# solufast-cvprojects/multigriddet

Hardware: NVIDIA B200
Metric: encode+decode/NMS images/sec, COCO 608×608, 1–8 B200; % HBM peak (higher is better)
Workload: dtype f32

## Files before the change

include/mgd.h:

```cpp
#ifndef MGD_H_
#define MGD_H_

#ifdef __cplusplus
extern "C" {
#endif

#if defined(__GNUC__)
#define MGD_API __attribute__((visibility("default")))
#else
#define MGD_API
#endif

#define MGD_VERSION 100
#define MGD_MAX_LAYERS 5
#define MGD_MAX_ANCHORS_PER_LAYER 8

typedef enum {
    MGD_OK = 0,
    MGD_ERR_INVALID_ARGUMENT = 1,
    MGD_ERR_CLASS_RANGE = 2,
    MGD_ERR_CUDA = 3,
    MGD_ERR_NO_DEVICE = 4,
    MGD_ERR_UNSUPPORTED = 5
} mgd_status;

enum { MGD_MEM_HOST = 0, MGD_MEM_DEVICE = 1 };

enum {
    MGD_FLAG_SYNC = 1,
    MGD_FLAG_HOST_ZEROCOPY = 4,
    MGD_FLAG_TF_COMPAT = 2
};

enum { MGD_NMS_IOU = 0, MGD_NMS_DIOU = 1, MGD_NMS_SOFT = 2, MGD_NMS_WBF = 3 };
enum { MGD_WBF_CONF_AVG = 0, MGD_WBF_CONF_MAX = 1, MGD_WBF_CONF_BOX_AND_MODEL_AVG = 2 };

typedef struct {
    int num_layers;
    int num_classes;
    int input_h, input_w;
    int grid_h[MGD_MAX_LAYERS];
    int grid_w[MGD_MAX_LAYERS];
    int num_anchors[MGD_MAX_LAYERS];
    double anchors[MGD_MAX_LAYERS][MGD_MAX_ANCHORS_PER_LAYER][2];
    int anchors_f64;
} mgd_head_config;

typedef struct {
    int use_softmax;
    int rescore_confidence;
    double confidence;
    double nms_threshold;
    int nms_method;
    int per_class;
    int max_boxes;
    double soft_sigma;
    double soft_score_threshold;
} mgd_post_config;

MGD_API int mgd_version(void);
MGD_API const char *mgd_last_error(void);
MGD_API int mgd_device_count(void);

MGD_API int mgd_encode_targets(const mgd_head_config *cfg, const float *boxes,
                       int batch, int max_boxes, float *const *y_true,
                       int memory, int device, void *stream, int flags,
                       long long *stats);

MGD_API int mgd_decode_nms(const mgd_head_config *cfg, const mgd_post_config *post,
                   const float *const *preds, int batch, const int *image_hw,
                   double *boxes_xywh, int *boxes_xyxy, double *scores,
                   int *classes, int *index, int *counts,
                   int memory, int device, void *stream, int flags,
                   long long *stats);

MGD_API int mgd_encode_decode_nms(const mgd_head_config *cfg, const mgd_post_config *post,
                          const float *gt_boxes, int enc_batch, int max_gt_boxes,
                          float *const *y_true,
                          const float *const *preds, int dec_batch, const int *image_hw,
                          double *boxes_xywh, int *boxes_xyxy, double *scores,
                          int *classes, int *index, int *counts,
                          int device, void *stream, int flags);

MGD_API int mgd_decode_dense(const mgd_head_config *cfg, const mgd_post_config *post,
                     const float *const *preds, int batch, const int *image_hw,
                     double *out, int memory, int device, void *stream, int flags);

MGD_API int mgd_nms(const double *boxes, const double *scores, const int *classes, int n,
            double nms_threshold, int nms_method, int per_class, int max_keep,
            int *keep, int *n_keep, int memory, int device, void *stream, int flags);

MGD_API int mgd_wbf(const double *boxes, const double *scores, const int *classes,
            const double *box_weights, int n, double iou_thr, double skip_box_thr,
            int conf_type, double *out_boxes, double *out_scores, int *out_classes,
            int *n_out, int memory, int device, void *stream, int flags);

MGD_API int mgd_soft_nms(const double *boxes, const double *scores, int n, double sigma,
                 double score_threshold, int *keep, double *soft_scores, int *n_keep,
                 int memory, int device, void *stream, int flags);

enum { MGD_IOU_CORNER = 0, MGD_IOU_CENTRE = 1 };
MGD_API int mgd_match_detections(const double *det_boxes, const double *det_scores,
                         const int *det_classes, const int *det_counts, int batch, int max_dets,
                         const double *gt_boxes, const int *gt_classes, const int *gt_counts,
                         int max_gt, const double *iou_thresholds, int num_thresholds,
                         int iou_mode, unsigned char *tp, int *matched_gt,
                         int memory, int device, void *stream, int flags);

MGD_API int mgd_ignore_mask(const mgd_head_config *cfg, const float *const *y_pred,
                    const float *const *y_true, int batch, double ignore_thresh, double eps,
                    float *const *ignore_mask, float *const *assigned_anchor_iou,
                    float *const *max_iou_map, int memory, int device, void *stream, int flags);

MGD_API int mgd_encode_ignore_mask(const mgd_head_config *cfg, const float *boxes, int batch,
                           int max_boxes, const float *const *y_pred, float *const *y_true,
                           double ignore_thresh, double eps, float *const *ignore_mask,
                           float *const *assigned_anchor_iou, float *const *max_iou_map,
                           int device, void *stream, int flags);

enum { MGD_BOXES_I32 = 0, MGD_BOXES_F64 = 1 };
MGD_API int mgd_reshape_boxes(const void *boxes, int boxes_dtype, const int *counts,
                      const int *params, int batch, int max_boxes, void *out, float *out_f32,
                      int *out_counts, int memory, int device, void *stream, int flags);
MGD_API int mgd_mosaic_merge_boxes(const double *boxes, int num_sources, int max_boxes,
                           const int *params, int batch, int height, int width, double *out,
                           float *out_f32, int *out_counts,
                           int memory, int device, void *stream, int flags);

MGD_API int mgd_letterbox_boxes(const float *boxes, const int *counts, const int *params,
                        int batch, int max_in, int input_h, int input_w,
                        int max_boxes_per_image, int expansion, float *out,
                        int memory, int device, void *stream, int flags);

MGD_API int mgd_iou_matrix(const double *boxes1, int n, const double *boxes2, int m, double *out,
                   int memory, int device, void *stream, int flags);

MGD_API int mgd_poll_status(int device, void *stream);

#include <stddef.h>
MGD_API int mgd_host_alloc(size_t bytes, void **ptr);
MGD_API int mgd_host_free(void *ptr);

#define MGD_IPC_HANDLE_BYTES 64
typedef struct mgd_exchange mgd_exchange;
MGD_API int mgd_exchange_create(int device, int world_size, int rank, size_t bytes,
                        mgd_exchange **exchange, unsigned char *handle);
MGD_API int mgd_exchange_connect(mgd_exchange *exchange, const unsigned char *handles);
MGD_API int mgd_exchange_buffer(mgd_exchange *exchange, void **base, size_t *bytes);
MGD_API int mgd_exchange_timeouts(mgd_exchange *exchange, void *stream, int *timeouts);
MGD_API int mgd_exchange_destroy(mgd_exchange *exchange);

MGD_API int mgd_release_workspace(void);

#define MGD_PROFILE_KINDS 5
MGD_API int mgd_profile_begin(void);
MGD_API int mgd_profile_end(double *ms, long long *launches);

struct DLTensor;
MGD_API int mgd_encode_targets_dlpack(const mgd_head_config *cfg, const struct DLTensor *boxes,
                              struct DLTensor *const *y_true, void *stream, int flags,
                              long long *stats);
MGD_API int mgd_decode_nms_dlpack(const mgd_head_config *cfg, const mgd_post_config *post,
                          const struct DLTensor *const *preds,
                          const struct DLTensor *image_hw,
                          struct DLTensor *boxes_xywh, struct DLTensor *boxes_xyxy,
                          struct DLTensor *scores, struct DLTensor *classes,
                          struct DLTensor *index, struct DLTensor *counts,
                          void *stream, int flags, long long *stats);

#ifdef __cplusplus
}
#endif
#endif
```

multigriddet_b200/_lib.py:

```python
from __future__ import annotations

import ctypes
import os

import numpy as np

_HERE = os.path.dirname(os.path.abspath(__file__))
LIB_PATH = os.path.join(_HERE, "libmgd.so")

MGD_MAX_LAYERS = 5
MGD_MAX_ANCHORS_PER_LAYER = 8
MEM_HOST, MEM_DEVICE = 0, 1
FLAG_SYNC = 1
FLAG_TF_COMPAT = 2
FLAG_HOST_ZEROCOPY = 4
NMS_IOU, NMS_DIOU, NMS_SOFT, NMS_WBF = 0, 1, 2, 3
IOU_CORNER, IOU_CENTRE = 0, 1
BOXES_I32, BOXES_F64 = 0, 1

OK, ERR_INVALID_ARGUMENT, ERR_CLASS_RANGE, ERR_CUDA, ERR_NO_DEVICE, ERR_UNSUPPORTED = range(6)


class HeadConfig(ctypes.Structure):
    _fields_ = [
        ("num_layers", ctypes.c_int),
        ("num_classes", ctypes.c_int),
        ("input_h", ctypes.c_int),
        ("input_w", ctypes.c_int),
        ("grid_h", ctypes.c_int * MGD_MAX_LAYERS),
        ("grid_w", ctypes.c_int * MGD_MAX_LAYERS),
        ("num_anchors", ctypes.c_int * MGD_MAX_LAYERS),
        ("anchors", ((ctypes.c_double * 2) * MGD_MAX_ANCHORS_PER_LAYER) * MGD_MAX_LAYERS),
        ("anchors_f64", ctypes.c_int),
    ]


class PostConfig(ctypes.Structure):
    _fields_ = [
        ("use_softmax", ctypes.c_int),
        ("rescore_confidence", ctypes.c_int),
        ("confidence", ctypes.c_double),
        ("nms_threshold", ctypes.c_double),
        ("nms_method", ctypes.c_int),
        ("per_class", ctypes.c_int),
        ("max_boxes", ctypes.c_int),
        ("soft_sigma", ctypes.c_double),
        ("soft_score_threshold", ctypes.c_double),
    ]


class MgdError(RuntimeError):
    pass


_lib = None

_FP = ctypes.POINTER(ctypes.c_float)
_DP = ctypes.POINTER(ctypes.c_double)
_IP = ctypes.POINTER(ctypes.c_int)
_LLP = ctypes.POINTER(ctypes.c_longlong)

EXPORTS = ("mgd_version", "mgd_last_error", "mgd_device_count", "mgd_encode_targets",
           "mgd_decode_nms", "mgd_decode_dense", "mgd_nms", "mgd_soft_nms", "mgd_wbf", "mgd_poll_status",
           "mgd_encode_targets_dlpack", "mgd_decode_nms_dlpack", "mgd_profile_begin",
           "mgd_profile_end", "mgd_match_detections", "mgd_iou_matrix", "mgd_host_alloc",
           "mgd_host_free", "mgd_release_workspace", "mgd_reshape_boxes", "mgd_mosaic_merge_boxes",
           "mgd_ignore_mask", "mgd_encode_decode_nms", "mgd_letterbox_boxes",
           "mgd_encode_ignore_mask", "mgd_exchange_create", "mgd_exchange_connect",
           "mgd_exchange_buffer", "mgd_exchange_timeouts", "mgd_exchange_destroy")

IPC_HANDLE_BYTES = 64


def load():
    global _lib
    if _lib is not None:
        return _lib
    if not os.path.isfile(LIB_PATH):
        raise MgdError(
            f"{LIB_PATH} not found: build it with `python -m multigriddet_b200.build` "
            "(needs nvcc).  multigriddet_b200 has no CPU fallback.")
    lib = ctypes.CDLL(LIB_PATH)
    lib.mgd_version.restype = ctypes.c_int
    lib.mgd_last_error.restype = ctypes.c_char_p
    lib.mgd_device_count.restype = ctypes.c_int
    lib.mgd_encode_targets.restype = ctypes.c_int
    lib.mgd_encode_targets.argtypes = [
        ctypes.POINTER(HeadConfig), ctypes.c_void_p, ctypes.c_int, ctypes.c_int,
        ctypes.POINTER(ctypes.c_void_p), ctypes.c_int, ctypes.c_int, ctypes.c_void_p,
        ctypes.c_int, _LLP]
    lib.mgd_decode_nms.restype = ctypes.c_int
    lib.mgd_decode_nms.argtypes = [
        ctypes.POINTER(HeadConfig), ctypes.POINTER(PostConfig),
        ctypes.POINTER(ctypes.c_void_p), ctypes.c_int, ctypes.c_void_p,
        ctypes.c_void_p, ctypes.c_void_p, ctypes.c_void_p, ctypes.c_void_p, ctypes.c_void_p,
        ctypes.c_void_p, ctypes.c_int, ctypes.c_int, ctypes.c_void_p, ctypes.c_int, _LLP]
    lib.mgd_encode_decode_nms.restype = ctypes.c_int
    lib.mgd_encode_decode_nms.argtypes = [
        ctypes.POINTER(HeadConfig), ctypes.POINTER(PostConfig),
        ctypes.c_void_p, ctypes.c_int, ctypes.c_int, ctypes.POINTER(ctypes.c_void_p),
        ctypes.POINTER(ctypes.c_void_p), ctypes.c_int, ctypes.c_void_p,
        ctypes.c_void_p, ctypes.c_void_p, ctypes.c_void_p, ctypes.c_void_p, ctypes.c_void_p,
        ctypes.c_void_p, ctypes.c_int, ctypes.c_void_p, ctypes.c_int]
    lib.mgd_decode_dense.restype = ctypes.c_int
    lib.mgd_decode_dense.argtypes = [
        ctypes.POINTER(HeadConfig), ctypes.POINTER(PostConfig),
        ctypes.POINTER(ctypes.c_void_p), ctypes.c_int, ctypes.c_void_p, ctypes.c_void_p,
        ctypes.c_int, ctypes.c_int, ctypes.c_void_p, ctypes.c_int]
    lib.mgd_nms.restype = ctypes.c_int
    lib.mgd_nms.argtypes = [
        ctypes.c_void_p, ctypes.c_void_p, ctypes.c_void_p, ctypes.c_int, ctypes.c_double,
        ctypes.c_int, ctypes.c_int, ctypes.c_int, ctypes.c_void_p, ctypes.c_void_p,
        ctypes.c_int, ctypes.c_int, ctypes.c_void_p, ctypes.c_int]
    lib.mgd_wbf.restype = ctypes.c_int
    lib.mgd_wbf.argtypes = [
        ctypes.c_void_p, ctypes.c_void_p, ctypes.c_void_p, ctypes.c_void_p, ctypes.c_int,
        ctypes.c_double, ctypes.c_double, ctypes.c_int, ctypes.c_void_p, ctypes.c_void_p,
        ctypes.c_void_p, ctypes.c_void_p, ctypes.c_int, ctypes.c_int, ctypes.c_void_p, ctypes.c_int]
    lib.mgd_soft_nms.restype = ctypes.c_int
    lib.mgd_soft_nms.argtypes = [
        ctypes.c_void_p, ctypes.c_void_p, ctypes.c_int, ctypes.c_double, ctypes.c_double,
        ctypes.c_void_p, ctypes.c_void_p, ctypes.c_void_p, ctypes.c_int, ctypes.c_int,
        ctypes.c_void_p, ctypes.c_int]
    lib.mgd_poll_status.restype = ctypes.c_int
    lib.mgd_poll_status.argtypes = [ctypes.c_int, ctypes.c_void_p]
    lib.mgd_encode_targets_dlpack.restype = ctypes.c_int
    lib.mgd_encode_targets_dlpack.argtypes = [
        ctypes.POINTER(HeadConfig), ctypes.c_void_p, ctypes.POINTER(ctypes.c_void_p),
        ctypes.c_void_p, ctypes.c_int, _LLP]
    lib.mgd_decode_nms_dlpack.restype = ctypes.c_int
    lib.mgd_decode_nms_dlpack.argtypes = [
        ctypes.POINTER(HeadConfig), ctypes.POINTER(PostConfig),
        ctypes.POINTER(ctypes.c_void_p), ctypes.c_void_p, ctypes.c_void_p, ctypes.c_void_p,
        ctypes.c_void_p, ctypes.c_void_p, ctypes.c_void_p, ctypes.c_void_p, ctypes.c_void_p,
        ctypes.c_int, _LLP]
    lib.mgd_match_detections.restype = ctypes.c_int
    lib.mgd_match_detections.argtypes = [
        ctypes.c_void_p, ctypes.c_void_p, ctypes.c_void_p, ctypes.c_void_p, ctypes.c_int, ctypes.c_int,
        ctypes.c_void_p, ctypes.c_void_p, ctypes.c_void_p, ctypes.c_int, _DP, ctypes.c_int,
        ctypes.c_int, ctypes.c_void_p, ctypes.c_void_p, ctypes.c_int, ctypes.c_int, ctypes.c_void_p,
        ctypes.c_int]
    lib.mgd_iou_matrix.restype = ctypes.c_int
    lib.mgd_iou_matrix.argtypes = [
        ctypes.c_void_p, ctypes.c_int, ctypes.c_void_p, ctypes.c_int, ctypes.c_void_p, ctypes.c_int,
        ctypes.c_int, ctypes.c_void_p, ctypes.c_int]
    lib.mgd_reshape_boxes.restype = ctypes.c_int
    lib.mgd_reshape_boxes.argtypes = [
        ctypes.c_void_p, ctypes.c_int, ctypes.c_void_p, ctypes.c_void_p, ctypes.c_int, ctypes.c_int,
        ctypes.c_void_p, ctypes.c_void_p, ctypes.c_void_p, ctypes.c_int, ctypes.c_int, ctypes.c_void_p,
        ctypes.c_int]
    lib.mgd_mosaic_merge_boxes.restype = ctypes.c_int
    lib.mgd_mosaic_merge_boxes.argtypes = [
        ctypes.c_void_p, ctypes.c_int, ctypes.c_int, ctypes.c_void_p, ctypes.c_int, ctypes.c_int,
        ctypes.c_int, ctypes.c_void_p, ctypes.c_void_p, ctypes.c_void_p, ctypes.c_int, ctypes.c_int,
        ctypes.c_void_p, ctypes.c_int]
    lib.mgd_encode_ignore_mask.restype = ctypes.c_int
    lib.mgd_encode_ignore_mask.argtypes = [
        ctypes.POINTER(HeadConfig), ctypes.c_void_p, ctypes.c_int, ctypes.c_int,
        ctypes.POINTER(ctypes.c_void_p), ctypes.POINTER(ctypes.c_void_p), ctypes.c_double, ctypes.c_double,
        ctypes.POINTER(ctypes.c_void_p), ctypes.POINTER(ctypes.c_void_p), ctypes.POINTER(ctypes.c_void_p),
        ctypes.c_int, ctypes.c_void_p, ctypes.c_int]
    lib.mgd_letterbox_boxes.restype = ctypes.c_int
    lib.mgd_letterbox_boxes.argtypes = [
        ctypes.c_void_p, ctypes.c_void_p, ctypes.c_void_p, ctypes.c_int, ctypes.c_int, ctypes.c_int,
        ctypes.c_int, ctypes.c_int, ctypes.c_int, ctypes.c_void_p, ctypes.c_int, ctypes.c_int,
        ctypes.c_void_p, ctypes.c_int]
    lib.mgd_ignore_mask.restype = ctypes.c_int
    lib.mgd_ignore_mask.argtypes = [
        ctypes.POINTER(HeadConfig), ctypes.POINTER(ctypes.c_void_p), ctypes.POINTER(ctypes.c_void_p),
        ctypes.c_int, ctypes.c_double, ctypes.c_double, ctypes.POINTER(ctypes.c_void_p),
        ctypes.POINTER(ctypes.c_void_p), ctypes.POINTER(ctypes.c_void_p), ctypes.c_int, ctypes.c_int,
        ctypes.c_void_p, ctypes.c_int]
    lib.mgd_host_alloc.restype = ctypes.c_int
    lib.mgd_host_alloc.argtypes = [ctypes.c_size_t, ctypes.POINTER(ctypes.c_void_p)]
    lib.mgd_host_free.restype = ctypes.c_int
    lib.mgd_host_free.argtypes = [ctypes.c_void_p]
    lib.mgd_release_workspace.restype = ctypes.c_int
    lib.mgd_exchange_create.restype = ctypes.c_int
    lib.mgd_exchange_create.argtypes = [ctypes.c_int, ctypes.c_int, ctypes.c_int, ctypes.c_size_t,
                                        ctypes.POINTER(ctypes.c_void_p), ctypes.c_void_p]
    lib.mgd_exchange_connect.restype = ctypes.c_int
    lib.mgd_exchange_connect.argtypes = [ctypes.c_void_p, ctypes.c_void_p]
    lib.mgd_exchange_buffer.restype = ctypes.c_int
    lib.mgd_exchange_buffer.argtypes = [ctypes.c_void_p, ctypes.POINTER(ctypes.c_void_p),
                                        ctypes.POINTER(ctypes.c_size_t)]
    lib.mgd_exchange_timeouts.restype = ctypes.c_int
    lib.mgd_exchange_timeouts.argtypes = [ctypes.c_void_p, ctypes.c_void_p, _IP]
    lib.mgd_exchange_destroy.restype = ctypes.c_int
    lib.mgd_exchange_destroy.argtypes = [ctypes.c_void_p]
    lib.mgd_profile_begin.restype = ctypes.c_int
    lib.mgd_profile_end.restype = ctypes.c_int
    lib.mgd_profile_end.argtypes = [_DP, _LLP]
    _lib = lib
    return lib


def raise_for_status(rc: int) -> None:
    if rc == OK:
        return
    msg = load().mgd_last_error().decode("utf-8", "replace")
    if rc == ERR_CLASS_RANGE:
        raise AssertionError(msg)
    if rc == ERR_INVALID_ARGUMENT:
        raise ValueError(msg)
    if rc == ERR_UNSUPPORTED:
        raise NotImplementedError(msg)
    raise MgdError(msg)


_cfg_cache: dict = {}


def make_head_config(anchors, num_classes, input_shape, grid_shapes=None) -> HeadConfig:
    arrs = [np.asarray(a) for a in anchors]
    key = (tuple((a.dtype.str, a.shape, a.tobytes()) for a in arrs), int(num_classes),
           int(input_shape[0]), int(input_shape[1]),
           None if grid_shapes is None else tuple((int(g[0]), int(g[1])) for g in grid_shapes))
    hit = _cfg_cache.get(key)
    if hit is not None:
        return hit
    cfg = _make_head_config(arrs, num_classes, input_shape, grid_shapes)
    if len(_cfg_cache) < 256:
        _cfg_cache[key] = cfg
    return cfg


def _make_head_config(arrs, num_classes, input_shape, grid_shapes=None) -> HeadConfig:
    num_layers = len(arrs)
    if not 1 <= num_layers <= MGD_MAX_LAYERS:
        raise ValueError(f"between 1 and {MGD_MAX_LAYERS} layers supported, got {num_layers}")
    cfg = HeadConfig()
    cfg.num_layers = num_layers
    cfg.num_classes = int(num_classes)
    cfg.input_h, cfg.input_w = int(input_shape[0]), int(input_shape[1])
    if grid_shapes is None:
        strides = (32, 16, 8, 4, 2)
        grid_shapes = [(cfg.input_h // strides[l], cfg.input_w // strides[l])
                       for l in range(num_layers)]
    f64 = False
    for l, a in enumerate(arrs):
        if a.ndim != 2 or a.shape[1] != 2 or not 1 <= a.shape[0] <= MGD_MAX_ANCHORS_PER_LAYER:
            raise ValueError(f"anchors[{l}] must have shape (1..{MGD_MAX_ANCHORS_PER_LAYER}, 2)")
        f64 = f64 or a.dtype == np.float64
        cfg.grid_h[l], cfg.grid_w[l] = int(grid_shapes[l][0]), int(grid_shapes[l][1])
        cfg.num_anchors[l] = a.shape[0]
        for i in range(a.shape[0]):
            cfg.anchors[l][i][0] = float(a[i, 0])
            cfg.anchors[l][i][1] = float(a[i, 1])
    cfg.anchors_f64 = int(f64)
    return cfg


def ptr_array(ptrs):
    return (ctypes.c_void_p * len(ptrs))(*[ctypes.c_void_p(int(p)) for p in ptrs])


class PinnedPool:

    def __init__(self, cap_bytes=None):
        import threading
        if cap_bytes is None:
            cap_bytes = int(os.environ.get("MGD_PINNED_CAP_MB", "4096")) << 20
        self._lock = threading.Lock()
        self._free = {}
        self._idle = 0
        self._total = 0
        self.cap_bytes = cap_bytes

    def _give_back(self, ptr, nbytes):
        with self._lock:
            self._free.setdefault(nbytes, []).append(ptr)
            self._idle += nbytes

    def _trim(self, need):
        victims = []
        with self._lock:
            for size in sorted(self._free, reverse=True):
                lst = self._free[size]
                while lst and self._total + need > self.cap_bytes:
                    victims.append(lst.pop())
                    self._idle -= size
                    self._total -= size
        for ptr in victims:
            load().mgd_host_free(ctypes.c_void_p(ptr))

    def empty(self, shape, dtype):
        import weakref
        dtype = np.dtype(dtype)
        nbytes = int(np.prod(shape, dtype=np.int64)) * dtype.itemsize
        if nbytes < (1 << 16):
            return np.empty(shape, dtype)
        ptr = None
        with self._lock:
            lst = self._free.get(nbytes)
            if lst:
                ptr = lst.pop()
                self._idle -= nbytes
        if ptr is None:
            if self._total + nbytes > self.cap_bytes:
                self._trim(nbytes)
            if self._total + nbytes > self.cap_bytes:
                return np.empty(shape, dtype)
            out = ctypes.c_void_p()
            if load().mgd_host_alloc(nbytes, ctypes.byref(out)) != OK or not out.value:
                return np.empty(shape, dtype)
            ptr = out.value
            with self._lock:
                self._total += nbytes
        buf = (ctypes.c_char * nbytes).from_address(ptr)
        weakref.finalize(buf, self._give_back, ptr, nbytes)
        return np.frombuffer(buf, dtype=dtype).reshape(shape)


pinned = PinnedPool()
```

multigriddet_b200/csrc/api.cu:

```cuda
#include <math.h>
#include <stdarg.h>
#include <stdio.h>
#include <string.h>

#include <chrono>
#include <functional>
#include <mutex>
#include <string>
#include <thread>
#include <vector>

#include "common.cuh"
#include "dlpack_abi.h"

namespace {

thread_local std::string t_error;

int fail(int code, const char* fmt, ...)
{
    char buf[512];
    va_list ap;
    va_start(ap, fmt);
    vsnprintf(buf, sizeof(buf), fmt, ap);
// ... 655 lines not shown
    {
        if (!s[0] && !s[1] && chunk[0].blocks.empty() && chunk[1].blocks.empty() &&
            call.blocks.empty() && !bounce[0] && !bounce[1]) return;
        for (int i = 0; i < 2; ++i) if (s[i]) cudaStreamSynchronize(s[i]);
        chunk[0].release(); chunk[1].release(); call.release();
        for (int i = 0; i < 2; ++i) {
            if (bounce[i]) cudaFreeHost(bounce[i]);
            if (bounce_done[i]) cudaEventDestroy(bounce_done[i]);
            if (ev[i]) cudaEventDestroy(ev[i]);
            if (s[i]) cudaStreamDestroy(s[i]);
        }
        cudaGetLastError();
    }
};
thread_local HostStreams t_streams[64];

int host_streams(int device, cudaStream_t** out, cudaEvent_t** ev, HostStreams** self = nullptr)
{
    HostStreams& hs = t_streams[device];
    if (self) *self = &hs;
    for (int i = 0; i < 2; ++i) {
        if (!hs.s[i]) CUDA_TRY(cudaStreamCreateWithFlags(&hs.s[i], cudaStreamNonBlocking));
        if (!hs.ev[i]) CUDA_TRY(cudaEventCreateWithFlags(&hs.ev[i], cudaEventDisableTiming));
    }
    *out = hs.s;
    if (ev) *ev = hs.ev;
    return MGD_OK;
}

bool is_pageable(const void* p)
{
    cudaPointerAttributes at;
    if (cudaPointerGetAttributes(&at, p) != cudaSuccess) { cudaGetLastError(); return true; }
    return at.type == cudaMemoryTypeUnregistered;
}

int host_copy_threads()
{
    static int n = -1;
    if (n < 0) {
        const char* e = getenv("MGD_HOST_COPY_THREADS");
        const int hw = (int)std::thread::hardware_concurrency();
        n = e ? atoi(e) : (hw >= 32 ? 8 : (hw >= 8 ? hw / 4 : 2));
        if (hw > 0 && n > hw) n = hw;
        if (n < 1) n = 1;
    }
    return n;
}

void parallel_copy(void* dst, const void* src, size_t bytes)
{
    const int n = bytes < (8u << 20) ? 1 : host_copy_threads();
    if (n == 1) { memcpy(dst, src, bytes); return; }
    const size_t part = ((bytes / n) + 4095) & ~(size_t)4095;
    std::vector<std::thread> workers;
    for (int i = 1; i < n; ++i) {
        const size_t off = (size_t)i * part;
        if (off >= bytes) break;
        const size_t len = off + part < bytes ? part : bytes - off;
        workers.emplace_back([=] { memcpy(static_cast<char*>(dst) + off, static_cast<const char*>(src) + off, len); });
    }
    memcpy(dst, src, part < bytes ? part : bytes);
    for (std::thread& t : workers) t.join();
}

int bounce_slot(HostStreams* hs, int slot, size_t bytes, unsigned char** out)
{
    if (hs->bounce_busy[slot]) {
        CUDA_TRY(cudaEventSynchronize(hs->bounce_done[slot]));
        hs->bounce_busy[slot] = false;
    }
    if (hs->bounce_cap[slot] < bytes) {
        if (hs->bounce[slot]) CUDA_TRY(cudaFreeHost(hs->bounce[slot]));
        hs->bounce[slot] = nullptr; hs->bounce_cap[slot] = 0;
        CUDA_TRY(cudaHostAlloc(reinterpret_cast<void**>(&hs->bounce[slot]), bytes, cudaHostAllocPortable));
        hs->bounce_cap[slot] = bytes;
    }
    if (!hs->bounce_done[slot]) CUDA_TRY(cudaEventCreateWithFlags(&hs->bounce_done[slot], cudaEventDisableTiming));
    *out = hs->bounce[slot];
    return MGD_OK;
}

template <typename T> T* mapped_alias(T* p, size_t bytes)
{
    if (!p || bytes == 0) return nullptr;
    const unsigned char* ends[2] = {reinterpret_cast<const unsigned char*>(p),
                                    reinterpret_cast<const unsigned char*>(p) + bytes - 1};
    void* dev = nullptr;
    for (int i = 0; i < 2; ++i) {
        cudaPointerAttributes at;
        if (cudaPointerGetAttributes(&at, ends[i]) != cudaSuccess) { cudaGetLastError(); return nullptr; }
        if (at.type != cudaMemoryTypeHost || !at.devicePointer) return nullptr;
        if (i == 0) dev = at.devicePointer;
    }
    return reinterpret_cast<T*>(dev);
}

int zerocopy_mode()
{
    static int v = -1;
    if (v < 0) { const char* e = getenv("MGD_HOST_ZEROCOPY"); v = e ? atoi(e) : 0; }
    return v;
}

int host_chunk(const HeadGeom& g, int batch)
{
    static long long mb = -1;
    if (mb < 0) { const char* e = getenv("MGD_HOST_CHUNK_MB"); mb = e && atoll(e) > 0 ? atoll(e) : 128; }
    long long per_image = 0;
    for (int l = 0; l < g.L; ++l) per_image += (long long)g.gh[l] * g.gw[l] * g.D[l] * 4;
    long long n = (mb << 20) / (per_image > 0 ? per_image : 1);
    if (n < 1) n = 1;
    if (n > batch) n = batch;
    return (int)n;
}

}

extern "C" {

int mgd_version(void) { return MGD_VERSION; }

const char* mgd_last_error(void) { return t_error.c_str(); }

int mgd_device_count(void) { return device_count_quiet(); }

int mgd_host_alloc(size_t bytes, void** ptr)
{
    if (!ptr) return fail(MGD_ERR_INVALID_ARGUMENT, "ptr is NULL");
    *ptr = nullptr;
    if (device_count_quiet() == 0)
        return fail(MGD_ERR_NO_DEVICE, "no CUDA device: page-locked memory is not available");
    CUDA_TRY(cudaHostAlloc(ptr, bytes ? bytes : 1, cudaHostAllocPortable));
    return MGD_OK;
}

int mgd_host_free(void* ptr)
{
    if (ptr) CUDA_TRY(cudaFreeHost(ptr));
    return MGD_OK;
}

int mgd_exchange_create(int device, int world_size, int rank, size_t bytes, mgd_exchange** out,
                        unsigned char* handle)
{
    if (!out || !handle) return fail(MGD_ERR_INVALID_ARGUMENT, "NULL argument");
    *out = nullptr;
    if (world_size < 1 || world_size > MGD_EXCHANGE_MAX_RANKS)
        return fail(MGD_ERR_UNSUPPORTED, "a detection exchange spans 1..%d ranks (one node), got %d",
                    MGD_EXCHANGE_MAX_RANKS, world_size);
    if (rank < 0 || rank >= world_size) return fail(MGD_ERR_INVALID_ARGUMENT, "rank %d outside [0, %d)", rank, world_size);
    if (bytes == 0) return fail(MGD_ERR_INVALID_ARGUMENT, "bytes must be > 0");
    int num_sms;
    DeviceScope dev_scope;
    int rc = prepare_device(device, &num_sms, &dev_scope);
    if (rc) return rc;
    static_assert(sizeof(cudaIpcMemHandle_t) == MGD_IPC_HANDLE_BYTES, "IPC handle size");
    mgd_exchange* ex = new mgd_exchange();
    ex->device = device;
    ex->world = world_size;
    ex->rank = rank;
    ex->bytes = (bytes + 255) & ~(size_t)255;
    void* p = nullptr;
    cudaError_t e = cudaMalloc(&p, MGD_EXCHANGE_HEADER_BYTES + ex->bytes);
    if (e == cudaSuccess) e = cudaMemset(p, 0, MGD_EXCHANGE_HEADER_BYTES + ex->bytes);
    if (e == cudaSuccess) e = cudaIpcGetMemHandle(&ex->handle, p);
    if (e != cudaSuccess) {
        if (p) cudaFree(p);
        delete ex;
        cudaGetLastError();
        return fail(MGD_ERR_CUDA, "exchange allocation failed: %s", cudaGetErrorString(e));
    }
    ex->alloc[rank] = static_cast<char*>(p);
    memcpy(handle, &ex->handle, MGD_IPC_HANDLE_BYTES);
    if (world_size == 1) {
        ex->connected = true;
        std::lock_guard<std::mutex> lock(g_exchange_mutex);
        g_exchanges.push_back(ex);
    }
    *out = ex;
    return MGD_OK;
}

int mgd_exchange_connect(mgd_exchange* ex, const unsigned char* handles)
{
    if (!ex || !handles) return fail(MGD_ERR_INVALID_ARGUMENT, "NULL argument");
    if (ex->connected) return MGD_OK;
    int num_sms;
    DeviceScope dev_scope;
    int rc = prepare_device(ex->device, &num_sms, &dev_scope);
    if (rc) return rc;
    for (int r = 0; r < ex->world; ++r) {
        if (r == ex->rank) continue;
        cudaIpcMemHandle_t h;
        memcpy(&h, handles + (size_t)r * MGD_IPC_HANDLE_BYTES, MGD_IPC_HANDLE_BYTES);
        void* p = nullptr;
        const cudaError_t e = cudaIpcOpenMemHandle(&p, h, cudaIpcMemLazyEnablePeerAccess);
        if (e != cudaSuccess) {
            for (int q = 0; q < r; ++q)
                if (q != ex->rank && ex->alloc[q]) { cudaIpcCloseMemHandle(ex->alloc[q]); ex->alloc[q] = nullptr; }
            cudaGetLastError();
            return fail(MGD_ERR_CUDA, "cannot map the exchange buffer of rank %d: %s (peer access over "
                        "NVLink / PCIe between the two devices is required)", r, cudaGetErrorString(e));
        }
        ex->alloc[r] = static_cast<char*>(p);
    }
    ex->connected = true;
    std::lock_guard<std::mutex> lock(g_exchange_mutex);
    g_exchanges.push_back(ex);
    return MGD_OK;
}

int mgd_exchange_buffer(mgd_exchange* ex, void** base, size_t* bytes)
{
    if (!ex || !base) return fail(MGD_ERR_INVALID_ARGUMENT, "NULL argument");
    *base = ex->alloc[ex->rank] + MGD_EXCHANGE_HEADER_BYTES;
    if (bytes) *bytes = ex->bytes;
    return MGD_OK;
}

int mgd_exchange_timeouts(mgd_exchange* ex, void* stream, int* timeouts)
{
    if (!ex || !timeouts) return fail(MGD_ERR_INVALID_ARGUMENT, "NULL argument");
    int num_sms;
    DeviceScope dev_scope;
    int rc = prepare_device(ex->device, &num_sms, &dev_scope);
    if (rc) return rc;
    unsigned v = 0;
    CUDA_TRY(cudaStreamSynchronize((cudaStream_t)stream));
    CUDA_TRY(cudaMemcpy(&v, reinterpret_cast<unsigned*>(ex->alloc[ex->rank]) + MGD_EXCHANGE_TIMEOUT_WORD,
                        sizeof(v), cudaMemcpyDeviceToHost));
    *timeouts = (int)v;
    return MGD_OK;
}

int mgd_exchange_destroy(mgd_exchange* ex)
{
    if (!ex) return MGD_OK;
    {
        std::lock_guard<std::mutex> lock(g_exchange_mutex);
        for (size_t i = 0; i < g_exchanges.size(); ++i)
            if (g_exchanges[i] == ex) { g_exchanges.erase(g_exchanges.begin() + i); break; }
    }
    int num_sms;
    DeviceScope dev_scope;
    if (prepare_device(ex->device, &num_sms, &dev_scope) == MGD_OK) {
        cudaDeviceSynchronize();
        for (int r = 0; r < ex->world; ++r) {
            if (!ex->alloc[r]) continue;
            if (r == ex->rank) cudaFree(ex->alloc[r]);
            else cudaIpcCloseMemHandle(ex->alloc[r]);
        }
        cudaGetLastError();
    }
    delete ex;
    return MGD_OK;
}

int mgd_release_workspace(void)
{
    int cur = 0;
    const bool have = cudaGetDevice(&cur) == cudaSuccess;
    for (int d = 0; d < 64; ++d) {
        HostStreams& hs = t_streams[d];
        if (hs.chunk[0].blocks.empty() && hs.chunk[1].blocks.empty() && hs.call.blocks.empty() &&
            !hs.bounce[0] && !hs.bounce[1]) continue;
        if (cudaSetDevice(d) != cudaSuccess) { cudaGetLastError(); continue; }
        for (int i = 0; i < 2; ++i) if (hs.s[i]) cudaStreamSynchronize(hs.s[i]);
        hs.chunk[0].release(); hs.chunk[1].release(); hs.call.release();
        for (int i = 0; i < 2; ++i) {
            if (hs.bounce[i]) cudaFreeHost(hs.bounce[i]);
            hs.bounce[i] = nullptr; hs.bounce_cap[i] = 0; hs.bounce_busy[i] = false;
        }
    }
    if (have) cudaSetDevice(cur);
    cudaGetLastError();
    return MGD_OK;
}

int mgd_profile_begin(void)
{
    for (ProfSpan& s : t_prof_spans) { cudaEventDestroy(s.t0); cudaEventDestroy(s.t1); }
    t_prof_spans.clear();
    t_prof_on = true;
    return MGD_OK;
}

int mgd_profile_end(double* ms, long long* launches)
{
    t_prof_on = false;
    for (int k = 0; k < PROF_KINDS; ++k) { if (ms) ms[k] = 0.0; if (launches) launches[k] = 0; }
    int rc = MGD_OK;
    for (ProfSpan& s : t_prof_spans) {
        float t = 0.f;
        cudaError_t e = cudaEventSynchronize(s.t1);
        if (e == cudaSuccess) e = cudaEventElapsedTime(&t, s.t0, s.t1);
        if (e != cudaSuccess) rc = fail(MGD_ERR_CUDA, "profile: %s", cudaGetErrorString(e));
        else { if (ms) ms[s.kind] += t; if (launches) launches[s.kind] += s.launches; }
        cudaEventDestroy(s.t0);
        cudaEventDestroy(s.t1);
    }
    t_prof_spans.clear();
    return rc;
}

int mgd_poll_status(int device, void* stream)
{
    int num_sms;
    DeviceScope dev_scope;
    int rc = prepare_device(device, &num_sms, &dev_scope);
    if (rc) return rc;
    CUDA_TRY(cudaStreamSynchronize((cudaStream_t)stream));
    int st = 0;
    if (t_deferred.word[device]) {
        CUDA_TRY(cudaMemcpy(&st, t_deferred.word[device], sizeof(int), cudaMemcpyDeviceToHost));
        if (st) CUDA_TRY(cudaMemset(t_deferred.word[device], 0, sizeof(int)));
    }
    return status_to_error(st);
}

int mgd_encode_targets(const mgd_head_config* cfg, const float* boxes, int batch, int max_boxes,
                       float* const* y_true, int memory, int device, void* stream, int flags,
                       long long* stats)
{
    nvtx_range nv_api("mgd_encode_targets");
    HeadGeom g;
    int rc = build_geom(cfg, &g);
    if (rc) return rc;
    if ((rc = check_memory_arg(memory))) return rc;
    if (batch < 0 || max_boxes < 0)
        return fail(MGD_ERR_INVALID_ARGUMENT, "batch and max_boxes must be >= 0");
    if (!y_true) return fail(MGD_ERR_INVALID_ARGUMENT, "y_true is NULL");
    for (int l = 0; l < g.L; ++l)
        if (!y_true[l] && batch > 0) return fail(MGD_ERR_INVALID_ARGUMENT, "y_true[%d] is NULL", l);
    if (!boxes && (long long)batch * max_boxes > 0)
        return fail(MGD_ERR_INVALID_ARGUMENT, "boxes is NULL");
    if (max_boxes > 65000)
        return fail(MGD_ERR_UNSUPPORTED, "max_boxes per image must be <= 65000, got %d", max_boxes);
    if ((long long)chunk_images(g, batch > 0 ? batch : 1) * max_boxes >= (1ll << 27))
        return fail(MGD_ERR_UNSUPPORTED, "batch chunk x max_boxes too large");
    int num_sms;
    DeviceScope dev_scope;
    if ((rc = prepare_device(device, &num_sms, &dev_scope))) return rc;
    if (stats) memset(stats, 0, 4 * sizeof(long long));
    if (batch == 0) return MGD_OK;

    if (memory == MGD_MEM_DEVICE && !(flags & MGD_FLAG_SYNC)) {
        cudaStream_t st = (cudaStream_t)stream;
        int* d_flag;
        if ((rc = deferred_status_word(device, &d_flag))) return rc;
        return encode_device(g, boxes, batch, max_boxes, y_true, num_sms, st, d_flag, nullptr,
                             Alloc{nullptr, st}, (flags & MGD_FLAG_TF_COMPAT) != 0);
    }
    if (memory == MGD_MEM_DEVICE) {
        cudaStream_t st = (cudaStream_t)stream;
        int* d_status;
        unsigned long long* d_stats = nullptr;
        CUDA_TRY(pool_malloc(&d_status, sizeof(int) + 4 * sizeof(unsigned long long), st));
        CUDA_TRY(cudaMemsetAsync(d_status, 0, sizeof(int) + 4 * sizeof(unsigned long long), st));
        d_stats = reinterpret_cast<unsigned long long*>(d_status);
        int* d_flag = reinterpret_cast<int*>(d_stats + 4);
        rc = encode_device(g, boxes, batch, max_boxes, y_true, num_sms, st, d_flag, d_stats,
                           Alloc{nullptr, st}, (flags & MGD_FLAG_TF_COMPAT) != 0);
        if (rc) return rc;
        if (flags & MGD_FLAG_SYNC) {
            unsigned long long h[5] = {0, 0, 0, 0, 0};
            CUDA_TRY(cudaMemcpyAsync(h, d_status, sizeof(int) + 4 * sizeof(unsigned long long),
                                     cudaMemcpyDeviceToHost, st));
            CUDA_TRY(cudaFreeAsync(d_status, st));
            CUDA_TRY(cudaStreamSynchronize(st));
            if (stats) for (int i = 0; i < 4; ++i) stats[i] = (long long)h[i];
            return status_to_error((int)(h[4] & 0xffffffffu));
        }
        CUDA_TRY(cudaFreeAsync(d_status, st));
        return MGD_OK;
    }

    Tracer tr("encode/host");
    cudaStream_t* ss;
    cudaEvent_t* ev;
    HostStreams* hs;
    if ((rc = host_streams(device, &ss, &ev, &hs))) return rc;
    hs->call.reset();
    unsigned long long* d_meta;
    CUDA_TRY(hs->call.take(reinterpret_cast<void**>(&d_meta), 5 * sizeof(unsigned long long)));
    CUDA_TRY(cudaMemsetAsync(d_meta, 0, 5 * sizeof(unsigned long long), ss[0]));
    float* d_boxes;
    const size_t box_bytes = (size_t)batch * max_boxes * 5 * sizeof(float);
    CUDA_TRY(hs->call.take(reinterpret_cast<void**>(&d_boxes), box_bytes));
    if (box_bytes) CUDA_TRY(cudaMemcpyAsync(d_boxes, boxes, box_bytes, cudaMemcpyHostToDevice, ss[0]));
    CUDA_TRY(cudaEventRecord(ev[0], ss[0]));
    CUDA_TRY(cudaStreamWaitEvent(ss[1], ev[0], 0));
    int step = host_chunk(g, batch);
    float* z_y[MGD_MAX_LAYERS];
    bool zero_copy = (zerocopy_mode() & 2) != 0 || (flags & MGD_FLAG_HOST_ZEROCOPY) != 0;
    for (int l = 0; l < g.L && zero_copy; ++l) {
        z_y[l] = mapped_alias(y_true[l], (size_t)batch * g.gh[l] * g.gw[l] * g.D[l] * 4);
        zero_copy = z_y[l] != nullptr;
    }
    if (zero_copy) step = batch;
    bool pageable = !zero_copy && host_copy_threads() > 1 &&
                    (size_t)batch * g.cells * g.D[0] * 4 >= (32u << 20);
    for (int l = 0; l < g.L && pageable; ++l) pageable = is_pageable(y_true[l]);
    struct CopyOut { bool live = false; size_t off[MGD_MAX_LAYERS], bytes[MGD_MAX_LAYERS]; float* dst[MGD_MAX_LAYERS]; };
    CopyOut pending[2];
    auto drain = [&](int slot) -> int {
        CopyOut& c = pending[slot];
        if (!c.live) return MGD_OK;
        CUDA_TRY(cudaEventSynchronize(hs->bounce_done[slot]));
        hs->bounce_busy[slot] = false;
        for (int l = 0; l < g.L; ++l) parallel_copy(c.dst[l], hs->bounce[slot] + c.off[l], c.bytes[l]);
        c.live = false;
        return MGD_OK;
    };
    int k = 0;
    for (int b0 = 0; b0 < batch; b0 += step, ++k) {
        const int nb = batch - b0 < step ? batch - b0 : step;
        cudaStream_t st = ss[k & 1];
        Arena& ar = hs->chunk[k & 1];
        ar.reset();
        float* d_y[MGD_MAX_LAYERS];
        for (int l = 0; l < g.L; ++l) {
            if (zero_copy) d_y[l] = z_y[l];
            else CUDA_TRY(ar.take(reinterpret_cast<void**>(&d_y[l]), (size_t)nb * g.gh[l] * g.gw[l] * g.D[l] * 4));
        }
        rc = encode_device(g, d_boxes + (size_t)b0 * max_boxes * 5, nb, max_boxes, d_y, num_sms, st,
                           reinterpret_cast<int*>(d_meta + 4), d_meta, Alloc{&ar, st},
                           (flags & MGD_FLAG_TF_COMPAT) != 0);
        if (rc) return rc;
        unsigned char* bounce = nullptr;
        if (pageable) {
            if ((rc = drain(k & 1))) return rc;
            size_t need = 0;
            for (int l = 0; l < g.L; ++l) need += (((size_t)nb * g.gh[l] * g.gw[l] * g.D[l] * 4) + 255) & ~(size_t)255;
            if ((rc = bounce_slot(hs, k & 1, need, &bounce))) return rc;
        }
        size_t bounce_off = 0;
        for (int l = 0; l < g.L && !zero_copy; ++l) {
            const size_t per = (size_t)g.gh[l] * g.gw[l] * g.D[l];
            const size_t bytes = (size_t)nb * per * 4;
            float* dst = y_true[l] + (size_t)b0 * per;
            if (bounce) {
                CopyOut& c = pending[k & 1];
                c.off[l] = bounce_off; c.bytes[l] = bytes; c.dst[l] = dst;
                dst = reinterpret_cast<float*>(bounce + bounce_off);
                bounce_off += (bytes + 255) & ~(size_t)255;
            }
            CUDA_TRY(cudaMemcpyAsync(dst, d_y[l], bytes, cudaMemcpyDeviceToHost, st));
        }
        if (bounce) {
            CUDA_TRY(cudaEventRecord(hs->bounce_done[k & 1], st));
            hs->bounce_busy[k & 1] = true;
            pending[k & 1].live = true;
        }
    }
    if (pageable) {
        if ((rc = drain(k & 1))) return rc;
        if ((rc = drain((k + 1) & 1))) return rc;
    }
    tr.mark("chunks enqueued");
    CUDA_TRY(cudaEventRecord(ev[1], ss[1]));
    CUDA_TRY(cudaStreamWaitEvent(ss[0], ev[1], 0));
    CUDA_TRY(cudaStreamSynchronize(ss[0]));
    unsigned long long h[5];
    CUDA_TRY(cudaMemcpy(h, d_meta, sizeof(h), cudaMemcpyDeviceToHost));
    tr.mark("synchronised");
    hs->chunk[0].consolidate(); hs->chunk[1].consolidate(); hs->call.consolidate();
    if (stats) for (int i = 0; i < 4; ++i) stats[i] = (long long)h[i];
    return status_to_error((int)(h[4] & 0xffffffffu));
}

int mgd_decode_nms(const mgd_head_config* cfg, const mgd_post_config* post,
                   const float* const* preds, int batch, const int* image_hw,
                   double* boxes_xywh, int* boxes_xyxy, double* scores, int* classes, int* index,
                   int* counts, int memory, int device, void* stream, int flags, long long* stats)
{
    nvtx_range nv_api("mgd_decode_nms");
    HeadGeom g;
    int rc = build_geom(cfg, &g);
    if (rc) return rc;
    if ((rc = check_post(post))) return rc;
    if ((rc = check_memory_arg(memory))) return rc;
    if (batch < 0) return fail(MGD_ERR_INVALID_ARGUMENT, "batch must be >= 0");
    if (!preds) return fail(MGD_ERR_INVALID_ARGUMENT, "preds is NULL");
    for (int l = 0; l < g.L; ++l)
        if (!preds[l] && batch > 0) return fail(MGD_ERR_INVALID_ARGUMENT, "preds[%d] is NULL", l);
    if (!counts && batch > 0) return fail(MGD_ERR_INVALID_ARGUMENT, "counts is NULL");
    int num_sms;
    DeviceScope dev_scope;
    if ((rc = prepare_device(device, &num_sms, &dev_scope))) return rc;
    if (stats) memset(stats, 0, 4 * sizeof(long long));
    if (batch == 0) return MGD_OK;
    const int M = post->max_boxes;

    if (memory == MGD_MEM_DEVICE) {
        cudaStream_t st = (cudaStream_t)stream;
        unsigned long long* d_stats = nullptr;
        const bool want_stats = stats && (flags & MGD_FLAG_SYNC);
        if (want_stats) {
            CUDA_TRY(pool_malloc(&d_stats, 4 * sizeof(unsigned long long), st));
            CUDA_TRY(cudaMemsetAsync(d_stats, 0, 4 * sizeof(unsigned long long), st));
        }
        rc = decode_nms_device(g, *post, preds, batch, image_hw, boxes_xywh, boxes_xyxy, scores,
                               classes, index, counts, num_sms, st, d_stats, Alloc{nullptr, st});
        if (rc) return rc;
        if (flags & MGD_FLAG_SYNC) {
            unsigned long long h[4] = {0, 0, 0, 0};
            if (want_stats) {
                CUDA_TRY(cudaMemcpyAsync(h, d_stats, sizeof(h), cudaMemcpyDeviceToHost, st));
                CUDA_TRY(cudaFreeAsync(d_stats, st));
            }
            CUDA_TRY(cudaStreamSynchronize(st));
            if (stats) for (int i = 0; i < 4; ++i) stats[i] = (long long)h[i];
        }
        return MGD_OK;
    }

    Tracer tr("decode_nms/host");
    cudaStream_t* ss;
    cudaEvent_t* ev;
    HostStreams* hs;
    if ((rc = host_streams(device, &ss, &ev, &hs))) return rc;
    tr.mark("streams");
    const size_t n_det = (size_t)batch * M;
    const size_t off_xywh = 4 * sizeof(unsigned long long);
    const size_t off_scores = off_xywh + n_det * 4 * sizeof(double);
    const size_t off_xyxy = off_scores + n_det * sizeof(double);
    const size_t off_cls = off_xyxy + n_det * 4 * sizeof(int);
    const size_t off_idx = off_cls + n_det * sizeof(int);
    const size_t off_cnt = off_idx + n_det * sizeof(int);
    const size_t off_hw = off_cnt + (size_t)batch * sizeof(int);
    const size_t slab = off_hw + (size_t)batch * 2 * sizeof(int);
    unsigned char* d_out;
    hs->call.reset();
    CUDA_TRY(hs->call.take(reinterpret_cast<void**>(&d_out), slab));
    unsigned long long* d_stats = reinterpret_cast<unsigned long long*>(d_out);
    CUDA_TRY(cudaMemsetAsync(d_stats, 0, 4 * sizeof(unsigned long long), ss[0]));
    int* d_hw = nullptr;
    if (image_hw) {
        d_hw = reinterpret_cast<int*>(d_out + off_hw);
        CUDA_TRY(cudaMemcpyAsync(d_hw, image_hw, (size_t)batch * 2 * sizeof(int), cudaMemcpyHostToDevice, ss[0]));
    }
    CUDA_TRY(cudaEventRecord(ev[0], ss[0]));
    CUDA_TRY(cudaStreamWaitEvent(ss[1], ev[0], 0));
    tr.mark("slab");
    int step = host_chunk(g, batch);
    const float* z_pred[MGD_MAX_LAYERS];
    bool zero_copy = (zerocopy_mode() & 1) != 0 || (flags & MGD_FLAG_HOST_ZEROCOPY) != 0;
    for (int l = 0; l < g.L && zero_copy; ++l) {
        z_pred[l] = mapped_alias(preds[l], (size_t)batch * g.gh[l] * g.gw[l] * g.D[l] * 4);
        zero_copy = z_pred[l] != nullptr;
    }
    bool pageable = !zero_copy && host_copy_threads() > 1 &&
                    (size_t)batch * g.cells * g.D[0] * 4 >= (32u << 20);
    for (int l = 0; l < g.L && pageable; ++l) pageable = is_pageable(preds[l]);
    int k = 0;
    for (int b0 = 0; b0 < batch; b0 += step, ++k) {
        const int nb = batch - b0 < step ? batch - b0 : step;
        cudaStream_t st = ss[k & 1];
        Arena& ar = hs->chunk[k & 1];
        ar.reset();
        float* d_pred[MGD_MAX_LAYERS];
        unsigned char* bounce = nullptr;
        size_t bounce_off = 0;
        if (pageable) {
            size_t need = 0;
            for (int l = 0; l < g.L; ++l) need += (((size_t)nb * g.gh[l] * g.gw[l] * g.D[l] * 4) + 255) & ~(size_t)255;
            if ((rc = bounce_slot(hs, k & 1, need, &bounce))) return rc;
        }
        for (int l = 0; l < g.L; ++l) {
            const size_t per = (size_t)g.gh[l] * g.gw[l] * g.D[l];
            if (zero_copy) { d_pred[l] = const_cast<float*>(z_pred[l]) + (size_t)b0 * per; continue; }
            const size_t bytes = (size_t)nb * per * 4;
            CUDA_TRY(ar.take(reinterpret_cast<void**>(&d_pred[l]), bytes));
            const void* src = preds[l] + (size_t)b0 * per;
            if (bounce) {
                parallel_copy(bounce + bounce_off, src, bytes);
                src = bounce + bounce_off;
                bounce_off += (bytes + 255) & ~(size_t)255;
            }
            CUDA_TRY(cudaMemcpyAsync(d_pred[l], src, bytes, cudaMemcpyHostToDevice, st));
        }
        if (bounce) {
            CUDA_TRY(cudaEventRecord(hs->bounce_done[k & 1], st));
            hs->bounce_busy[k & 1] = true;
        }
        rc = decode_nms_device(g, *post, d_pred, nb, d_hw ? d_hw + 2 * (size_t)b0 : nullptr,
                               reinterpret_cast<double*>(d_out + off_xywh) + (size_t)b0 * M * 4,
                               reinterpret_cast<int*>(d_out + off_xyxy) + (size_t)b0 * M * 4,
                               reinterpret_cast<double*>(d_out + off_scores) + (size_t)b0 * M,
                               reinterpret_cast<int*>(d_out + off_cls) + (size_t)b0 * M,
                               reinterpret_cast<int*>(d_out + off_idx) + (size_t)b0 * M,
                               reinterpret_cast<int*>(d_out + off_cnt) + b0, num_sms, st, d_stats,
                               Alloc{&ar, st});
        if (rc) return rc;
    }
    tr.mark("chunks enqueued");
    CUDA_TRY(cudaEventRecord(ev[1], ss[1]));
    CUDA_TRY(cudaStreamWaitEvent(ss[0], ev[1], 0));
    cudaStream_t st = ss[0];
    CUDA_TRY(cudaStreamSynchronize(st));
    unsigned long long h[4];
    CUDA_TRY(cudaMemcpyAsync(h, d_stats, sizeof(h), cudaMemcpyDeviceToHost, st));
    if (boxes_xywh)
        CUDA_TRY(cudaMemcpyAsync(boxes_xywh, d_out + off_xywh, n_det * 4 * sizeof(double), cudaMemcpyDeviceToHost, st));
    if (scores)
// ... 927 lines not shown
```

multigriddet_b200/csrc/common.cuh:

```cuda
#pragma once
#include <cuda_runtime.h>
#include <stdint.h>
#include "../../include/mgd.h"

#define MGD_MAX_TOTAL_ANCHORS (MGD_MAX_LAYERS * MGD_MAX_ANCHORS_PER_LAYER)

struct HeadGeom {
    int L, C;
    int in_h, in_w;
    int gh[MGD_MAX_LAYERS], gw[MGD_MAX_LAYERS];
    int na[MGD_MAX_LAYERS];
    int D[MGD_MAX_LAYERS];
    int anchor_first[MGD_MAX_LAYERS];
    int K;
    int cell_off[MGD_MAX_LAYERS];
    int cells;
    int anchors_f64;
    float anc32[MGD_MAX_TOTAL_ANCHORS][2];
    double anc64[MGD_MAX_TOTAL_ANCHORS][2];
};

struct __align__(16) BoxRec {
    double fx, fy;
    float tw, th;
    int hot_anchor;
    int hot_class;
};

struct EncodeArgs {
    HeadGeom g;
    int B, N;
    const float* boxes;
    float* y[MGD_MAX_LAYERS];
    int* table;
    int* big_tables;
    BoxRec* recs;
    int tf_compat;
    int* status;
    unsigned long long* stats;
};

struct __align__(16) Cand {
    float score;
    int index;
    float t[4];
    int cls;
    int anchor;
};

struct __align__(16) BoxD { double x, y, w, h; };

struct DecodeArgs {
    HeadGeom g;
    int B;
    const float* pred[MGD_MAX_LAYERS];
    const int* image_hw;
    int use_softmax, rescore;
    double confidence;
    float obj_logit_min;
    float score_lo;
    long long rows_in_layer[MGD_MAX_LAYERS];
    unsigned long long cells_magic[MGD_MAX_LAYERS];
    Cand* cand;
    int* counts;
    int chunk_blocks;
    int debug;
};

#define MGD_MAX_MIRRORS 7
struct NmsArgs {
    HeadGeom g;
    int B;
    int cap;
    const Cand* cand;
    const double* in_boxes;
    const double* in_scores;
    const int* in_classes;
    BoxD* boxes;
    const int* counts;
    const int* image_hw;
    int in_h, in_w;
    double thr;
    int use_diou, per_class, max_boxes;
    int skip_small;
    int soft;
    double soft_sigma, soft_thr;
    double* soft_scratch;
    int wbf;
    int wbf_conf_type;
    const double* in_weights;
    int* wbf_ints;
    int* next_image;
    unsigned long long* sort_scratch;
    int sort_scratch_stride;
    unsigned char* kept_scratch;
    size_t kept_scratch_stride;
    double* out_xywh; int* out_xyxy; double* out_scores; int* out_classes; int* out_index;
    int* out_counts;
    unsigned long long* stats;
    int n_mirrors;
    long long mirror_delta[MGD_MAX_MIRRORS];
    int warp_ctas_per_sm;
};

#define MGD_EXCHANGE_MAX_RANKS 8
#define MGD_EXCHANGE_HEADER_BYTES 512
#define MGD_EXCHANGE_TIMEOUT_WORD 32
struct ExchangeView {
    int world, rank;
    unsigned* header[MGD_EXCHANGE_MAX_RANKS];
};
enum { MGD_EXCHANGE_SIGNAL = 1, MGD_EXCHANGE_WAIT = 2 };
cudaError_t launch_exchange_barrier(const ExchangeView& v, int which, unsigned epoch, int phase,
                                    cudaStream_t stream);

#define MGD_MAX_IOU_THRESHOLDS 16
struct MatchArgs {
    int B, M, N, T;
    const double* det_boxes;
    const double* det_scores;
    const int* det_classes;
    const int* det_counts;
    const double* gt_boxes;
    const int* gt_classes;
    const int* gt_counts;
    double thr[MGD_MAX_IOU_THRESHOLDS];
    int mode;
    unsigned char* tp;
    int* matched;
    int* next_image;
};

struct BoxOpArgs {
    int B, N;
    const void* in;
    const int* counts;
    const int* params;
    int n_src, height, width;
    void* out;
    float* out_f32;
    int* out_counts;
};

struct LossArgs {
    HeadGeom g;
    int B;
    const float* y_pred[MGD_MAX_LAYERS];
    const float* y_true[MGD_MAX_LAYERS];
    float ignore_thresh, eps;
    float* ignore[MGD_MAX_LAYERS];
    float* assigned[MGD_MAX_LAYERS];
    float* max_iou[MGD_MAX_LAYERS];
    void* gt_boxes;
    float* gt_area;
    int* gt_count;
    const int* table;
    const BoxRec* recs;
};

#include <nvtx3/nvToolsExt.h>
struct nvtx_range {
    explicit nvtx_range(const char* name) { nvtxRangePushA(name); }
    ~nvtx_range() { nvtxRangePop(); }
    nvtx_range(const nvtx_range&) = delete;
    nvtx_range& operator=(const nvtx_range&) = delete;
};

enum ProfKind { PROF_ENCODE_ASSIGN = 0, PROF_ENCODE_FILL = 1, PROF_DECODE_COMPACT = 2,
                PROF_NMS = 3, PROF_OTHER = 4, PROF_KINDS = 5 };
void prof_mark_begin(int kind, cudaStream_t stream);
void prof_mark_end(int kind, cudaStream_t stream);
void prof_group_begin(int kind, cudaStream_t stream);
void prof_group_end(int kind, cudaStream_t stream);

cudaError_t launch_encode(const EncodeArgs& a, int num_sms, cudaStream_t stream);
cudaError_t launch_encode_assign(const EncodeArgs& a, cudaStream_t stream,
                                 bool overlap_previous = false);
cudaError_t launch_encode_fill(const EncodeArgs& a, int num_sms, cudaStream_t stream,
                               bool overlap_previous = false);
cudaError_t launch_decode(const DecodeArgs& a, int num_sms, cudaStream_t stream);
cudaError_t launch_nms(const NmsArgs& a, int num_sms, cudaStream_t stream);
size_t encode_assign_smem_bytes(const HeadGeom& g, int N);
bool encode_needs_big_tables(const HeadGeom& g, int N);
int nms_smem_capacity();
size_t nms_kept_bytes(int max_boxes);
cudaError_t launch_decode_dense(const DecodeArgs& a, const int* image_hw, double* out,
                                cudaStream_t stream);
cudaError_t launch_match(const MatchArgs& a, int num_sms, cudaStream_t stream);
cudaError_t launch_iou_matrix(const double* b1, int n, const double* b2, int m, double* out,
                              cudaStream_t stream);
cudaError_t launch_reshape_boxes(const BoxOpArgs& a, int boxes_i32, cudaStream_t stream);
cudaError_t launch_mosaic_merge(const BoxOpArgs& a, cudaStream_t stream);
cudaError_t launch_letterbox_boxes(const float* in, const int* counts, const int* params, int B,
                                   int n_in, int n_keep, int capacity, int input_h, int input_w,
                                   float* out, cudaStream_t stream);
cudaError_t launch_ignore_mask(const LossArgs& a, cudaStream_t stream);
cudaError_t launch_keep_from_index(const int* index, const int* counts, int max_keep, int* keep,
                                   int* n_keep, cudaStream_t stream);
```

multigriddet_b200/csrc/decode.cu:

```cuda
#include <math.h>
#include <stdlib.h>
#include <string.h>
#include "common.cuh"
#include "decode_math.cuh"

namespace {

constexpr int kWarpsPerCta = 8;
constexpr int kThreads = kWarpsPerCta * 32;
constexpr int kDenseThreads = 256;

__device__ __forceinline__ uint32_t smem_u32(const void* p)
{
    return (uint32_t)__cvta_generic_to_shared(p);
}
__device__ __forceinline__ void mbar_init(uint64_t* bar, uint32_t count)
{
    asm volatile("mbarrier.init.shared::cta.b64 [%0], %1;" ::"r"(smem_u32(bar)), "r"(count));
}
__device__ __forceinline__ void fence_mbar_init()
{
    asm volatile("fence.mbarrier_init.release.cluster;" ::: "memory");
}
__device__ __forceinline__ void mbar_expect_tx(uint64_t* bar, uint32_t bytes)
// ... 30 lines not shown
    uint64_t* bar;
    int stride;
};

template <bool kFast, int kPoolRows>
__device__ __noinline__ void flush_pool(const DecodeArgs& a, const WarpPool& pool, int count,
                                        int layer, const uint64_t* s_tab)
{
    const HeadGeom& g = a.g;
    const int lane = threadIdx.x & 31;
    const int A = g.na[layer], C = g.C;
    const bool softmax = a.use_softmax != 0;
    const bool rescore = a.rescore != 0;

    bool pass = lane < count;
    if (pass && rescore) {
        const float* c = pool.rows + lane * pool.stride + 5 + A;
        float mc = -INFINITY, sum = 0.f;
        if (kFast) {
            const float4* c4 = reinterpret_cast<const float4*>(c);
            #pragma unroll 4
            for (int i = 0; i < C / 4; ++i) {
                const float4 v = c4[i];
                mc = fmaxf(fmaxf(mc, fmaxf(v.x, v.y)), fmaxf(v.z, v.w));
                if (softmax) sum += (fast_exp(v.x) + fast_exp(v.y)) + (fast_exp(v.z) + fast_exp(v.w));
            }
        } else {
            for (int i = 0; i < C; ++i) {
                mc = fmaxf(mc, c[i]);
                if (softmax) sum += fast_exp(c[i]);
            }
        }
        float ub;
        if (softmax) {
            ub = __fdividef(pool.bound[lane] * fast_exp(mc), sum);
            if (!(sum < 3.0e38f) || !(ub == ub)) ub = 3.0e38f;
        } else {
            ub = pool.bound[lane] * fast_sigmoid(mc);
        }
        pass = ub >= a.score_lo;
    }
    unsigned todo = __ballot_sync(0xffffffffu, pass);

    const int j = lane & 7;
    const int oct = lane >> 3;
    const unsigned omask = 0xffu << (oct * 8);
    const int cells_l = g.gh[layer] * g.gw[layer];
    while (todo) {
        const unsigned pos = nth_set_bit(todo, oct);
        if (pos < 32u) {
            float* x = pool.rows + pos * pool.stride;
            float pa, pc; int ka, kc;
            octet_probs(x + 5, A, j, omask, softmax, s_tab, pa, ka);
            octet_probs(x + 5 + A, C, j, omask, softmax, s_tab, pc, kc);
            float score = mgd_expitf_tab(x[4], s_tab);
            if (rescore) score = __fmul_rn(__fmul_rn(score, pa), pc);
            if (j == 0 && (double)score >= a.confidence) {
                const int grow = pool.cell[pos];
                const int b = grow / cells_l;
                const int cell = grow - b * cells_l;
                Cand cd;
                cd.score = score;
                cd.index = g.cell_off[layer] + cell;
                cd.t[0] = x[0]; cd.t[1] = x[1]; cd.t[2] = x[2]; cd.t[3] = x[3];
                cd.cls = kc;
                cd.anchor = g.anchor_first[layer] + ka;
                const int slot = atomicAdd(a.counts + b, 1);
                a.cand[(size_t)b * g.cells + slot] = cd;
            }
        }
        __syncwarp();
        #pragma unroll
        for (int q = 0; q < 4; ++q) todo &= todo - 1;
    }
    if (kFast) asm volatile("fence.proxy.async.shared::cta;" ::: "memory");
    __syncwarp();
}

template <bool kFast, int kPoolRows>
__global__ void __launch_bounds__(kThreads, kPoolRows >= 32 ? 2 : (kPoolRows >= 24 ? 3 : (kPoolRows >= 16 ? 4 : 2)))
decode_compact_kernel(const __grid_constant__ DecodeArgs a, int pool_stride)
{
    extern __shared__ __align__(128) unsigned char smem_raw[];
    __shared__ uint64_t s_bar[kWarpsPerCta];
    __shared__ uint64_t s_tab[MGD_EXP2F_N];
    __shared__ int s_cell[kWarpsPerCta][kPoolRows];
    __shared__ float s_bound[kWarpsPerCta][kPoolRows];

    const HeadGeom& g = a.g;
    const int tid = threadIdx.x;
    const int lane = tid & 31;
    const int warp = tid >> 5;
    WarpPool pool;
    pool.rows = reinterpret_cast<float*>(smem_raw) + (size_t)warp * kPoolRows * pool_stride;
    pool.cell = s_cell[warp];
    pool.bound = s_bound[warp];
    pool.bar = &s_bar[warp];
    pool.stride = pool_stride;

    if (tid < MGD_EXP2F_N) s_tab[tid] = mgd_exp2f_tab[tid];
    if (kFast && lane == 0) {
        mbar_init(pool.bar, 1);
        fence_mbar_init();
    }
    __syncthreads();

    const int gwarp = blockIdx.x * kWarpsPerCta + warp;
    const int n_warps = gridDim.x * kWarpsPerCta;
    const bool softmax = a.use_softmax != 0;
    const bool rescore = a.rescore != 0;
    uint32_t bar_phase = 0;

    for (int layer = 0; layer < g.L; ++layer) {
        const int D = g.D[layer];
        const int A = g.na[layer];
        const int n_rows = (int)a.rows_in_layer[layer];
        const int n_blocks = (n_rows + 31) >> 5;
        const float* base = a.pred[layer];
        int count = 0;

        auto load_head = [&](int blk, float4& q) {
            const int row = blk * 32 + lane;
            q = make_float4(NAN, 0.f, 0.f, 0.f);
            if (blk < n_blocks && row < n_rows) {
                if (kFast) q = __ldg(reinterpret_cast<const float4*>(base + (size_t)row * D + 4));
                else q.x = __ldg(base + (size_t)row * D + 4);
            }
        };
        float4 q_next;
        load_head(gwarp, q_next);
        for (int blk = gwarp; blk < n_blocks; blk += n_warps) {
            const float4 q = q_next;
            load_head(blk + n_warps, q_next);
            const int row = blk * 32 + lane;

            float bound = 0.f;
            bool pass = false;
            if (q.x >= a.obj_logit_min) {
                bound = fast_sigmoid(q.x);
                if (rescore) {
                    if (kFast) {
                        const float ma = fmaxf(q.y, fmaxf(q.z, q.w));
                        if (softmax)
                            bound = __fdividef(bound, (fast_exp(q.y - ma) + fast_exp(q.z - ma)) + fast_exp(q.w - ma));
                        else
                            bound *= fast_sigmoid(ma);
                    } else {
                        const float* an = base + (size_t)row * D + 5;
                        float ma = __ldg(an);
                        for (int i = 1; i < A; ++i) ma = fmaxf(ma, __ldg(an + i));
                        if (softmax) {
                            float sa = 0.f;
                            for (int i = 0; i < A; ++i) sa += fast_exp(__ldg(an + i) - ma);
                            bound = __fdividef(bound, sa);
                        } else {
                            bound *= fast_sigmoid(ma);
                        }
                    }
                }
                pass = bound >= a.score_lo;
            }
            unsigned todo = __ballot_sync(0xffffffffu, pass);
            if (!todo) continue;

            while (todo) {
                const int free_slots = kPoolRows - count;
                const int rank = __popc(todo & ((1u << lane) - 1u));
                const bool take = ((todo >> lane) & 1u) && rank < free_slots;
                const unsigned taken = __ballot_sync(0xffffffffu, take);
                const int n_new = __popc(taken);
                if (take) {
                    pool.cell[count + rank] = row;
                    pool.bound[count + rank] = bound;
                }
                if (kFast) {
                    if (lane == 0) mbar_expect_tx(pool.bar, (uint32_t)n_new * D * sizeof(float));
                    __syncwarp();
                    if (take)
                        bulk_g2s(pool.rows + (size_t)(count + rank) * pool.stride,
                                 base + (size_t)row * D, (uint32_t)D * sizeof(float), pool.bar);
                } else {
                    unsigned rest = taken;
                    int slot = count;
                    while (rest) {
                        const int src_lane = __ffs((int)rest) - 1;
                        rest &= rest - 1;
                        const float* src = base + ((size_t)blk * 32 + src_lane) * D;
                        float* dst = pool.rows + (size_t)slot * pool.stride;
                        for (int i = lane; i < D; i += 32) dst[i] = __ldg(src + i);
                        ++slot;
                    }
                    __syncwarp();
                }
                count += n_new;
                todo &= ~taken;
                if (count == kPoolRows) {
                    if (kFast) {
                        if (lane == 0) mbar_arrive(pool.bar);
                        mbar_wait(pool.bar, bar_phase);
                        bar_phase ^= 1u;
                    }
                    flush_pool<kFast, kPoolRows>(a, pool, count, layer, s_tab);
                    count = 0;
                }
            }
        }
        if (count) {
            if (kFast) {
                if (lane == 0) mbar_arrive(pool.bar);
                mbar_wait(pool.bar, bar_phase);
                bar_phase ^= 1u;
            }
            flush_pool<kFast, kPoolRows>(a, pool, count, layer, s_tab);
        }
        __syncwarp();
    }
}

namespace ws {

template <int kProducers_, int kConsumers_, int kSlots_, int kRows_ = 32, int kPrefetch_ = 16>
struct Shape {
    static constexpr int kPrefetch = kPrefetch_;
    static constexpr int kProducers = kProducers_;
    static constexpr int kConsumers = kConsumers_;
    static constexpr int kThreads = (kProducers_ + kConsumers_) * 32;
    static constexpr int kSlots = kSlots_;
    static constexpr int kRows = kRows_;
    static constexpr int kCtasPerSm = kSlots_ * kRows_ > 9 * 32 ? 1 : 2;
};
constexpr int kSlotRows = 32;

struct SlotMeta {
    int row[kSlotRows];
    float bound[kSlotRows];
    int count;
    int layer;
    int pad[2];
};

__device__ __forceinline__ float expf_core2(float x, const uint32_t* tab)
{
    const double inv_ln2_n = 0x1.71547652b82fep+0 * MGD_EXP2F_N;
    const double shift = 0x1.8p+52;
    const double c0 = 0x1.c6af84b912394p-5 / MGD_EXP2F_N / MGD_EXP2F_N / MGD_EXP2F_N;
    const double c1 = 0x1.ebfce50fac4f3p-3 / MGD_EXP2F_N / MGD_EXP2F_N;
    const double c2 = 0x1.62e42ff0c52d6p-1 / MGD_EXP2F_N;
    const double z = __dmul_rn(inv_ln2_n, (double)x);
    double kd = __dadd_rn(z, shift);
    const int ki = __double2loint(kd);
    kd = __dsub_rn(kd, shift);
    const double r = __fma_rn(inv_ln2_n, (double)x, -kd);
    const int idx = ki & (MGD_EXP2F_N - 1);
    const int hi = (int)tab[idx + MGD_EXP2F_N] + (ki << 15);
    const double sc = __hiloint2double(hi, (int)tab[idx]);
    const double q = __fma_rn(c0, r, c1);
    const double r2 = __dmul_rn(r, r);
    double y = __fma_rn(c2, r, 1.0);
    y = __fma_rn(q, r2, y);
    y = __dmul_rn(y, sc);
    return __double2float_rn(y);
}

__device__ __forceinline__ float expf_full2(float x, const uint32_t* tab)
{
    float special = 0.f;
    bool is_special = false;
    if (!(x < 88.0f && x > -88.0f)) {
        if (x != x) { special = x + x; is_special = true; }
        else if (x > 88.72283172607421875f) { special = __builtin_huge_valf(); is_special = true; }
        else if (x < -103.972076416015625f) { special = 0.0f; is_special = true; }
    }
    const float v = expf_core2(is_special ? 0.f : x, tab);
    return is_special ? special : v;
}

__device__ __forceinline__ void near_track(float d, float thr, int i, int& first, int& cnt)
{
    asm("{\n .reg .pred p;\n setp.ge.f32 p, %2, %3;\n @p min.s32 %0, %0, %4;\n @p add.s32 %1, %1, 1;\n}"
        : "+r"(first), "+r"(cnt) : "f"(d), "f"(thr), "r"(i));
}

__device__ __forceinline__ int ld_acquire_smem(const int* p)
{
    int v;
    asm volatile("ld.acquire.cta.shared.s32 %0, [%1];" : "=r"(v) : "r"(smem_u32(p)) : "memory");
    return v;
}
__device__ __forceinline__ void st_release_smem(int* p, int v)
{
    asm volatile("st.release.cta.shared.s32 [%0], %1;" ::"r"(smem_u32(p)), "r"(v) : "memory");
}

struct GroupShared {
    float4* stage;
    float* rows;
    SlotMeta* meta;
    uint64_t* full;
    int* published;
    int* released;
    int* fill_seq;
    int* next_seq;
    int* producers_done;
    int stride;
};

template <class Sh>
__device__ __forceinline__ void producer(const DecodeArgs& a, const GroupShared& gs, int p, int P)
{
    constexpr int kSlots = Sh::kSlots;
    constexpr int kRows = Sh::kRows;
    constexpr int kPrefetch = Sh::kPrefetch;
    constexpr int kConsumers = Sh::kConsumers;
    constexpr int kProducers = Sh::kProducers;
    const HeadGeom& g = a.g;
    const int lane = threadIdx.x & 31;
    const bool softmax = a.use_softmax != 0;
    const bool rescore = a.rescore != 0;
    int seq = 0, slot = 0, count = 0;
    bool have_slot = false;

    auto acquire = [&]() {
        if (lane == 0) {
            seq = atomicAdd(gs.fill_seq, 1);
            const int use = seq / kSlots;
            while (ld_acquire_smem(&gs.released[seq % kSlots]) != use) __nanosleep(40);
        }
        seq = __shfl_sync(0xffffffffu, seq, 0);
        slot = seq % kSlots;
        have_slot = true;
    };
    auto publish = [&](int cnt, int layer) {
        if (lane == 0) { gs.meta[slot].count = cnt; gs.meta[slot].layer = layer; }
        __syncwarp();
        if (lane == 0) {
            mbar_arrive(&gs.full[slot]);
            st_release_smem(&gs.published[slot], seq);
        }
        have_slot = false;
        count = 0;
    };

    for (int layer = 0; layer < g.L; ++layer) {
        const int D = g.D[layer];
        const int n_rows = (int)a.rows_in_layer[layer];
        const int n_blocks = (n_rows + 31) >> 5;
        const float* base = a.pred[layer];
        auto issue_head = [&](int blk, int st) {
            const int row = blk * 32 + lane;
            if (blk < n_blocks && row < n_rows)
                asm volatile("cp.async.cg.shared.global [%0], [%1], 16;"
                             ::"r"(smem_u32(gs.stage + st * 32 + lane)), "l"(base + (size_t)row * D + 4) : "memory");
            asm volatile("cp.async.commit_group;" ::: "memory");
        };
        const int kChunk = a.chunk_blocks;
        #pragma unroll
        for (int k = 0; k < kPrefetch; ++k) issue_head((p + (k / kChunk) * P) * kChunk + k % kChunk, k);
        auto stage_rows = [&](int blk, unsigned todo, float bound) {
            const int row = blk * 32 + lane;
            while (todo) {
                if (!have_slot) acquire();
                const int free_slots = kRows - count;
                const int rank = __popc(todo & ((1u << lane) - 1u));
                const bool take = ((todo >> lane) & 1u) && rank < free_slots;
                const unsigned taken = __ballot_sync(0xffffffffu, take);
                const int n_new = __popc(taken);
                if (take) {
                    gs.meta[slot].row[count + rank] = row;
                    gs.meta[slot].bound[count + rank] = bound;
                }
                if (lane == 0) mbar_expect_tx(&gs.full[slot], (uint32_t)n_new * D * sizeof(float));
                __syncwarp();
                if (take)
                    bulk_g2s(gs.rows + ((size_t)slot * kRows + count + rank) * gs.stride,
                             base + (size_t)row * D, (uint32_t)D * sizeof(float), &gs.full[slot]);
                count += n_new;
                todo &= ~taken;
                if (count == kRows) publish(count, layer);
            }
        };
        int st = 0;
        for (int chunk = p; chunk * kChunk < n_blocks; chunk += P) {
            for (int u = 0; u < kChunk; ++u) {
                const int blk = chunk * kChunk + u;
                asm volatile("cp.async.wait_group %0;" ::"n"(kPrefetch - 1) : "memory");
                const int row = blk * 32 + lane;
                float4 h = gs.stage[st * 32 + lane];
                if (row >= n_rows) h.x = NAN;
                issue_head(blk + kPrefetch * P, st);
                st = st + 1 == kPrefetch ? 0 : st + 1;

                float bound = 0.f;
                bool pass = false;
                if (h.x >= a.obj_logit_min) {
                    bound = fast_sigmoid(h.x);
                    if (rescore) {
                        const float ma = fmaxf(h.y, fmaxf(h.z, h.w));
                        if (softmax)
                            bound = __fdividef(bound, (fast_exp(h.y - ma) + fast_exp(h.z - ma)) + fast_exp(h.w - ma));
                        else
                            bound *= fast_sigmoid(ma);
                    }
                    pass = bound >= a.score_lo;
                }
                unsigned todo = __ballot_sync(0xffffffffu, pass);
                if (a.debug & 1) todo = 0;
                stage_rows(blk, todo, bound);
            }
        }
        if (count) publish(count, layer);
    }
    int done = 0;
    if (lane == 0) done = atomicAdd(gs.producers_done, 1) + 1;
    done = __shfl_sync(0xffffffffu, done, 0);
    if (done == kProducers)
        for (int c = 0; c < kConsumers; ++c) {
            acquire();
            publish(-1, 0);
        }
}

template <class Sh, int kC>
__device__ __forceinline__ void consumer(const DecodeArgs& a, const GroupShared& gs,
                                         const uint32_t* tab)
{
    constexpr int kSlots = Sh::kSlots;
    constexpr int kRows = Sh::kRows;
    constexpr int kSplit = 32 / kRows;
    const HeadGeom& g = a.g;
    const int lane = threadIdx.x & 31;
    const int j = lane & 7;
    const int oct = lane >> 3;
    const bool softmax = a.use_softmax != 0;
    const bool rescore = a.rescore != 0;
    const int C = kC ? kC : g.C;
    const int body = C >= 8 ? (C & ~7) : 0;
    const int tail = C - body;
    constexpr float kNear = 0.99999f;
    constexpr float kNearD = -1.1e-5f;

    for (;;) {
        int seq = 0;
        if (lane == 0) {
            seq = atomicAdd(gs.next_seq, 1);
            while (ld_acquire_smem(&gs.published[seq % kSlots]) != seq) __nanosleep(40);
        }
        seq = __shfl_sync(0xffffffffu, seq, 0);
        const int slot = seq % kSlots;
        mbar_wait(&gs.full[slot], ((unsigned)(seq / kSlots)) & 1u);
        const SlotMeta& meta = gs.meta[slot];
        const int count = meta.count;
        if (count < 0) break;
        const int layer = meta.layer;
        const float* rows = gs.rows + (size_t)slot * kRows * gs.stride;

        const int lrow = lane & (kRows - 1), part = lane / kRows;
        bool pass = lrow < count && !(a.debug & 4);
        float mc = -INFINITY, sum = 0.f;
        if (pass) {
            const float4* c4 = reinterpret_cast<const float4*>(rows + (size_t)lrow * gs.stride + 8);
            const int n4 = C / 4, per = (n4 + kSplit - 1) / kSplit;
            const int i0 = part * per, i1 = min(n4, i0 + per);
            if (softmax && rescore) {
                #pragma unroll 4
                for (int i = i0; i < i1; ++i) {
                    const float4 v = c4[i];
                    mc = fmaxf(fmaxf(mc, fmaxf(v.x, v.y)), fmaxf(v.z, v.w));
                    sum += (fast_exp(v.x) + fast_exp(v.y)) + (fast_exp(v.z) + fast_exp(v.w));
                }
            } else {
                #pragma unroll 4
                for (int i = i0; i < i1; ++i) {
                    const float4 v = c4[i];
                    mc = fmaxf(fmaxf(mc, fmaxf(v.x, v.y)), fmaxf(v.z, v.w));
                }
            }
        }
        if (kSplit == 2) {
            mc = fmaxf(mc, __shfl_xor_sync(0xffffffffu, mc, 16));
            sum += __shfl_xor_sync(0xffffffffu, sum, 16);
        }
        if (pass && rescore) {
            if (softmax) {
                float ub = __fdividef(meta.bound[lrow] * fast_exp(mc), sum);
                if (!(sum < 3.0e38f) || !(ub == ub)) ub = 3.0e38f;
                pass = ub >= a.score_lo;
            } else {
                pass = meta.bound[lrow] * fast_sigmoid(mc) >= a.score_lo;
            }
        }
        unsigned todo = __ballot_sync(0xffffffffu, pass) & (kRows == 32 ? 0xffffffffu : (1u << (kRows & 31)) - 1u);
        if (a.debug & 2) todo = 0;

        unsigned cand_rows = 0;
        while (todo) {
            const unsigned pos = nth_set_bit(todo, oct);
            const bool live = pos < 32u;
            const unsigned posr = live ? pos : (unsigned)__ffs((int)todo) - 1u;
            const float* x = rows + (size_t)posr * gs.stride;
            const float mx = __shfl_sync(0xffffffffu, mc, (int)posr);
            const float4 head = *reinterpret_cast<const float4*>(x + 4);
            const int l0 = oct * 8;
            float pa, pc, obj;
            int ka, kc;
            if (softmax) {
                const float ma = fmaxf(head.y, fmaxf(head.z, head.w));
                const float logit = x[5 + (j < 2 ? j : 2)];
                const float da = __fsub_rn(logit, ma);
                const float arg = j < 3 ? (da < -104.0f ? -104.0f : da) : (j == 3 ? -head.x : 0.f);
                const float ea = expf_full2(arg, tab);

                const float* cx = x + 8;
                float r = 0.f, e_tail = 0.f;
                int near_cnt = 0, near_first = INT_MAX;
                if (body) {
                    #pragma unroll 10
                    for (int i = j; i < body; i += 8) {
                        const float d = __fsub_rn(cx[i], mx);
                        const float e = expf_core2(d < -104.0f ? -104.0f : d, tab);
                        r = __fadd_rn(r, e);
                        near_track(d, kNearD, i, near_first, near_cnt);
                    }
                    r = __fadd_rn(r, __shfl_xor_sync(0xffffffffu, r, 1));
                    r = __fadd_rn(r, __shfl_xor_sync(0xffffffffu, r, 2));
                    r = __fadd_rn(r, __shfl_xor_sync(0xffffffffu, r, 4));
                }
                if (tail) {
                    if (j < tail) {
                        const float d = __fsub_rn(cx[body + j], mx);
                        e_tail = expf_core2(d < -104.0f ? -104.0f : d, tab);
                        near_track(d, kNearD, body + j, near_first, near_cnt);
                    }
                    for (int k = 0; k < tail; ++k)
                        r = __fadd_rn(r, __shfl_sync(0xffffffffu, e_tail, l0 + k));
                }
                pc = __frcp_rn(r);
                const float e0 = __shfl_sync(0xffffffffu, ea, l0);
                const float e1 = __shfl_sync(0xffffffffu, ea, l0 + 1);
                const float e2 = __shfl_sync(0xffffffffu, ea, l0 + 2);
                const float eo = __shfl_sync(0xffffffffu, ea, l0 + 3);
                const float sa = __fadd_rn(__fadd_rn(__fadd_rn(0.f, e0), e1), e2);
                pa = __frcp_rn(sa);
                obj = __frcp_rn(__fadd_rn(1.0f, eo));
                const unsigned has = (__ballot_sync(0xffffffffu, near_cnt > 0) >> l0) & 0xffu;
                const unsigned many = (__ballot_sync(0xffffffffu, near_cnt > 1) >> l0) & 0xffu;
                const bool simple = !many && __popc(has) == 1;
                kc = __shfl_sync(0xffffffffu, near_first, l0 + (has ? __ffs((int)has) - 1 : 0));
                const int n0 = e0 >= kNear, n1 = e1 >= kNear, n2 = e2 >= kNear;
                ka = n0 ? 0 : (n1 ? 1 : 2);
                if (__any_sync(0xffffffffu, !simple || n0 + n1 + n2 != 1)) {
                    int first = INT_MAX;
                    for (int i = j; i < C; i += 8) {
                        const float d = __fsub_rn(cx[i], mx);
                        const float e = expf_core2(d < -104.0f ? -104.0f : d, tab);
                        if (e >= kNear && __fdiv_rn(e, r) == pc) { first = i; break; }
                    }
                    first = min(first, __shfl_xor_sync(0xffffffffu, first, 1));
                    first = min(first, __shfl_xor_sync(0xffffffffu, first, 2));
                    first = min(first, __shfl_xor_sync(0xffffffffu, first, 4));
                    if (!simple) kc = first;
                    if (n0 + n1 + n2 != 1) {
                        ka = INT_MAX;
                        if (n2 && __fdiv_rn(e2, sa) == pa) ka = 2;
                        if (n1 && __fdiv_rn(e1, sa) == pa) ka = 1;
                        if (n0 && __fdiv_rn(e0, sa) == pa) ka = 0;
                    }
                }
            } else {
                float best = -INFINITY;
                int first = INT_MAX;
                for (int i = j; i < C; i += 8) {
                    const float qv = __fdiv_rn(1.0f, __fadd_rn(1.0f, expf_full2(-x[8 + i], tab)));
                    if (qv > best) { best = qv; first = i; }
                }
                #pragma unroll
                for (int d = 1; d <= 4; d <<= 1) {
                    const float ob = __shfl_xor_sync(0xffffffffu, best, d);
                    const int oi = __shfl_xor_sync(0xffffffffu, first, d);
                    if (ob > best || (ob == best && oi < first)) { best = ob; first = oi; }
                }
                pc = best; kc = first;
                const float logit = j == 0 ? head.x : (j == 1 ? head.y : (j == 2 ? head.z : head.w));
                const float qv = __fdiv_rn(1.0f, __fadd_rn(1.0f, expf_full2(-logit, tab)));
                obj = __shfl_sync(0xffffffffu, qv, l0);
                const float q0 = __shfl_sync(0xffffffffu, qv, l0 + 1);
                const float q1 = __shfl_sync(0xffffffffu, qv, l0 + 2);
                const float q2 = __shfl_sync(0xffffffffu, qv, l0 + 3);
                pa = -INFINITY; ka = INT_MAX;
                if (q0 > pa) { pa = q0; ka = 0; }
                if (q1 > pa) { pa = q1; ka = 1; }
                if (q2 > pa) { pa = q2; ka = 2; }
            }
            float score = obj;
            if (rescore) score = __fmul_rn(__fmul_rn(score, pa), pc);
            const bool is_cand = live && j == 0 && (double)score >= a.confidence;
            __syncwarp();
            if (is_cand) {
                float4 res;
                res.x = score;
                res.y = __int_as_float(kc);
                res.z = __int_as_float(g.anchor_first[layer] + ka);
                res.w = 0.f;
                *reinterpret_cast<float4*>(const_cast<float*>(x) + 4) = res;
            }
            cand_rows |= __reduce_or_sync(0xffffffffu, is_cand ? (1u << pos) : 0u);
            #pragma unroll
            for (int q = 0; q < 4; ++q) todo &= todo - 1;
        }
        __syncwarp();
        const bool mine = lane < kRows && ((cand_rows >> lane) & 1u);
        float4 t = make_float4(0.f, 0.f, 0.f, 0.f), res = t;
        unsigned grow = 0;
        if (mine) {
            const float* x = rows + (size_t)lane * gs.stride;
            t = *reinterpret_cast<const float4*>(x);
            res = *reinterpret_cast<const float4*>(x + 4);
            grow = (unsigned)meta.row[lane];
        }
        if (cand_rows) asm volatile("fence.proxy.async.shared::cta;" ::: "memory");
        __syncwarp();
        if (lane == 0) st_release_smem(&gs.released[slot], seq / kSlots + 1);
        if (cand_rows) {
            const unsigned long long magic = a.cells_magic[layer];
            const unsigned b = magic ? (unsigned)__umul64hi((unsigned long long)grow, magic) : grow;
            const unsigned same = __match_any_sync(0xffffffffu, mine ? b : (0x80000000u | (unsigned)lane));
            const int leader = __ffs((int)same) - 1;
            int base = 0;
            if (mine && lane == leader) base = atomicAdd(a.counts + b, __popc(same));
            base = __shfl_sync(0xffffffffu, base, leader);
            if (mine) {
                Cand cd;
                cd.score = res.x;
                cd.index = g.cell_off[layer] + (int)(grow - b * (unsigned)(g.gh[layer] * g.gw[layer]));
                cd.t[0] = t.x; cd.t[1] = t.y; cd.t[2] = t.z; cd.t[3] = t.w;
                cd.cls = __float_as_int(res.y);
                cd.anchor = __float_as_int(res.z);
                a.cand[(size_t)b * g.cells + base + __popc(same & ((1u << lane) - 1u))] = cd;
            }
        }
    }
}

template <class Sh, int kC>
__global__ void __launch_bounds__(Sh::kThreads, Sh::kCtasPerSm)
decode_ws_kernel(const __grid_constant__ DecodeArgs a, int stride)
{
    constexpr int kSlots = Sh::kSlots, kProducers = Sh::kProducers;
    extern __shared__ __align__(128) unsigned char smem_raw[];
    __shared__ uint64_t s_full[kSlots];
    __shared__ int s_published[kSlots], s_released[kSlots];
    __shared__ SlotMeta s_meta[kSlots];
    __shared__ uint32_t s_tab[2 * MGD_EXP2F_N];
    __shared__ int s_counters[3];


    const int tid = threadIdx.x;
    const int warp = tid >> 5;
    if (tid < MGD_EXP2F_N) {
        s_tab[tid] = (uint32_t)mgd_exp2f_tab[tid];
        s_tab[tid + MGD_EXP2F_N] = (uint32_t)(mgd_exp2f_tab[tid] >> 32);
    }
    if (tid == 0) {
        for (int sl = 0; sl < kSlots; ++sl) {
            mbar_init(&s_full[sl], 1);
            s_published[sl] = -1;
            s_released[sl] = 0;
        }
        s_counters[0] = s_counters[1] = s_counters[2] = 0;
        fence_mbar_init();
    }
    __syncthreads();

    GroupShared gs;
    gs.rows = reinterpret_cast<float*>(smem_raw);
    constexpr int kFirstProducer = Sh::kConsumers;
    const int pw = warp - kFirstProducer;
    gs.stage = reinterpret_cast<float4*>(gs.rows + (size_t)kSlots * Sh::kRows * stride) +
               (size_t)(pw >= 0 ? pw : 0) * Sh::kPrefetch * 32;
    gs.meta = s_meta;
    gs.full = s_full;
    gs.published = s_published;
    gs.released = s_released;
    gs.fill_seq = &s_counters[0];
    gs.next_seq = &s_counters[1];
    gs.producers_done = &s_counters[2];
    gs.stride = stride;
    if (pw >= 0)
        producer<Sh>(a, gs, blockIdx.x * kProducers + pw, gridDim.x * kProducers);
    else
        consumer<Sh, kC>(a, gs, s_tab);
}

}

__global__ void __launch_bounds__(kDenseThreads, 3)
decode_dense_kernel(const __grid_constant__ DecodeArgs a, const int* image_hw, double* out,
                    int row_floats)
{
    extern __shared__ __align__(128) unsigned char smem_raw[];
    __shared__ uint64_t s_tab[MGD_EXP2F_N];
    const HeadGeom& g = a.g;
    const int tid = threadIdx.x, j = tid & 7;
    const unsigned omask = 0xffu << (((tid & 31) >> 3) * 8);
    float* x = reinterpret_cast<float*>(smem_raw) + (size_t)(tid >> 3) * row_floats;
    if (tid < MGD_EXP2F_N) s_tab[tid] = mgd_exp2f_tab[tid];
    __syncthreads();
    const long long total_rows = (long long)a.B * g.cells;
    const long long octs = (long long)gridDim.x * (kDenseThreads / 8);
    const long long iters = (total_rows + octs - 1) / octs;
    for (long long it = 0; it < iters; ++it) {
        long long q = it * octs + (long long)blockIdx.x * (kDenseThreads / 8) + (tid >> 3);
        const bool live = q < total_rows;
        if (!live) q = total_rows - 1;
        const int b = (int)(q / g.cells);
        const int flat = (int)(q - (long long)b * g.cells);
        int layer = 0;
        while (layer + 1 < g.L && flat >= g.cell_off[layer + 1]) ++layer;
        const int cell = flat - g.cell_off[layer];
        const int D = g.D[layer], A = g.na[layer];
        const float* src = a.pred[layer] + ((size_t)b * g.gh[layer] * g.gw[layer] + cell) * D;
        for (int i = j; i < D; i += 8) x[i] = __ldg(src + i);
        __syncwarp(omask);
        float pa, pc; int ka, kc;
        octet_probs(x + 5, A, j, omask, a.use_softmax != 0, s_tab, pa, ka);
        octet_probs(x + 5 + A, g.C, j, omask, a.use_softmax != 0, s_tab, pc, kc);
        __syncwarp(omask);
        float score = mgd_expitf_tab(x[4], s_tab);
        if (a.rescore) score = __fmul_rn(__fmul_rn(score, pa), pc);
        const int rr = cell / g.gw[layer], cc = cell - rr * g.gw[layer];
        double box[4];
        Letterbox lb;
        if (image_hw) lb = letterbox_consts(g.in_h, g.in_w, image_hw[2 * b], image_hw[2 * b + 1]);
        decode_axis_of(g, x, layer, g.anchor_first[layer] + ka, rr, cc, image_hw ? &lb : nullptr, 0,
                       s_tab, box[0], box[2]);
        decode_axis_of(g, x, layer, g.anchor_first[layer] + ka, rr, cc, image_hw ? &lb : nullptr, 1,
                       s_tab, box[1], box[3]);
        if (live) {
            double* o = out + (size_t)q * (5 + g.C);
            if (j < 4) o[j] = box[j];
            if (j == 4) o[4] = (double)score;
            float s = 1.0f;
            if (a.use_softmax) s = np_sum_octet(x + 5 + A, g.C, j, omask);
            for (int i = j; i < g.C; i += 8) {
                const float e = x[5 + A + i];
                o[5 + i] = (double)(a.use_softmax ? __fdiv_rn(e, s) : e);
            }
        } else if (a.use_softmax) {
            (void)np_sum_octet(x + 5 + A, g.C, j, omask);
        }
        __syncwarp(omask);
    }
}

}

cudaError_t launch_decode(const DecodeArgs& a_in, int num_sms, cudaStream_t stream)
{
    DecodeArgs a = a_in;
    const HeadGeom& g = a.g;
    int dmax = 0;
    bool fast = true;
    for (int l = 0; l < g.L; ++l) {
        dmax = g.D[l] > dmax ? g.D[l] : dmax;
        fast = fast && g.na[l] == 3 && (g.D[l] % 4 == 0) &&
               ((reinterpret_cast<uintptr_t>(a.pred[l]) & 15) == 0);
        a.rows_in_layer[l] = (long long)a.B * g.gh[l] * g.gw[l];
        if (a.rows_in_layer[l] >= 0x7fffffffll - 64) return cudaErrorInvalidValue;
        const unsigned long long cells_l = (unsigned long long)g.gh[l] * g.gw[l];
        a.cells_magic[l] = cells_l > 1 ? ~0ull / cells_l + 1ull : 0ull;
    }
    int stride = fast ? (dmax / 4 | 1) * 4 : (dmax | 1);
    if (fast && stride < dmax) stride += 8;

    static int env_impl = -1;
    static int env_shape = 0;
    if (env_impl < 0) {
        const char* e = getenv("MGD_DECODE_IMPL");
        env_impl = e && !strcmp(e, "legacy") ? 1 : 0;
        const char* sh = getenv("MGD_DECODE_SHAPE");
        env_shape = sh ? atoi(sh) : 0;
    }
    static int env_debug = -1;
    if (env_debug < 0) { const char* e = getenv("MGD_DECODE_DEBUG"); env_debug = e ? atoi(e) : 0; }
    a.debug = env_debug;
    if (fast && g.C <= 128 && !env_impl) {
        long long blocks = 0;
        for (int l = 0; l < g.L; ++l) blocks += (a.rows_in_layer[l] + 31) / 32;
        const int ws_stride = dmax;
        auto run = [&](auto shape) -> cudaError_t {
            using Sh = decltype(shape);
            const size_t smem = (size_t)Sh::kSlots * Sh::kRows * ws_stride * sizeof(float) +
                                (size_t)Sh::kProducers * Sh::kPrefetch * 32 * sizeof(float4);
            const size_t fixed = 1024 + 1024 + (size_t)Sh::kSlots * 304;
            int ctas_per_sm = (int)((227 * 1024) / (smem + fixed));
            if (ctas_per_sm > Sh::kCtasPerSm) ctas_per_sm = Sh::kCtasPerSm;
            if (ctas_per_sm < 1) return cudaErrorInvalidConfiguration;
            long long grid = (long long)num_sms * ctas_per_sm;
            const long long needed = (blocks + Sh::kProducers * 4 - 1) / (Sh::kProducers * 4);
            if (grid > needed) grid = needed;
            if (grid < 1) grid = 1;
            const long long per_producer = blocks / (grid * Sh::kProducers);
            a.chunk_blocks = per_producer >= 768 ? 8 : (per_producer >= 64 ? 2 : 1);
            static int env_cb = -1;
            if (env_cb < 0) { const char* e = getenv("MGD_DECODE_CHUNK_BLOCKS"); env_cb = e ? atoi(e) : 0; }
            if (env_cb == 1 || env_cb == 2 || env_cb == 4 || env_cb == 8) a.chunk_blocks = env_cb;

            auto kernel = g.C == 80 ? ws::decode_ws_kernel<Sh, 80> : ws::decode_ws_kernel<Sh, 0>;
            cudaError_t e = cudaFuncSetAttribute(kernel, cudaFuncAttributeMaxDynamicSharedMemorySize, (int)smem);
            if (e != cudaSuccess) return e;
            prof_mark_begin(PROF_DECODE_COMPACT, stream);
            kernel<<<(unsigned)grid, Sh::kThreads, smem, stream>>>(a, ws_stride);
            prof_mark_end(PROF_DECODE_COMPACT, stream);
            return cudaGetLastError();
        };
        cudaError_t err;
        if (env_shape == 1) err = run(ws::Shape<3, 6, 17, 16, 8>());
        else if (env_shape == 3) err = run(ws::Shape<3, 8, 17, 16, 8>());
        else if (env_shape == 4) err = run(ws::Shape<3, 6, 7, 32>());
        else if (env_shape == 5) err = run(ws::Shape<2, 4, 8, 32>());
        else err = run(ws::Shape<3, 7, 17, 16, 8>());
        if (err != cudaErrorInvalidConfiguration) return err;
        cudaGetLastError();
    }
    static int env_pool = -1;
    if (env_pool < 0) { const char* e = getenv("MGD_DECODE_POOL_ROWS"); env_pool = e ? atoi(e) : 0; }
    int pool_rows = env_pool == 32 || env_pool == 24 || env_pool == 16 ? env_pool : 32;
    while (pool_rows > 16 && (size_t)kWarpsPerCta * pool_rows * stride * sizeof(float) > 200 * 1024) pool_rows -= 8;
    while (pool_rows > 4 && (size_t)kWarpsPerCta * pool_rows * stride * sizeof(float) > 200 * 1024) pool_rows /= 2;
    const size_t smem = (size_t)kWarpsPerCta * pool_rows * stride * sizeof(float);
    if (smem > 220 * 1024) return cudaErrorInvalidConfiguration;
    int ctas_per_sm = (int)((224 * 1024) / (smem + 2048));
    const int reg_limit = pool_rows >= 32 ? 2 : (pool_rows >= 24 ? 3 : (pool_rows >= 16 ? 4 : 2));
    if (ctas_per_sm > reg_limit) ctas_per_sm = reg_limit;
    if (ctas_per_sm < 1) ctas_per_sm = 1;
    long long blocks = 0;
    for (int l = 0; l < g.L; ++l) blocks += (a.rows_in_layer[l] + 31) / 32;
    long long grid = (long long)num_sms * ctas_per_sm;
    const long long needed = (blocks + kWarpsPerCta - 1) / kWarpsPerCta;
    if (grid > needed) grid = needed;
    if (grid < 1) grid = 1;
    cudaError_t err;
    prof_mark_begin(PROF_DECODE_COMPACT, stream);
    auto run = [&](auto kernel) -> cudaError_t {
        cudaError_t e = cudaFuncSetAttribute(kernel, cudaFuncAttributeMaxDynamicSharedMemorySize, (int)smem);
        if (e != cudaSuccess) return e;
        kernel<<<(unsigned)grid, kThreads, smem, stream>>>(a, stride);
        return cudaSuccess;
    };
    if (fast) {
        if (pool_rows == 32) err = run(decode_compact_kernel<true, 32>);
        else if (pool_rows == 24) err = run(decode_compact_kernel<true, 24>);
        else if (pool_rows == 16) err = run(decode_compact_kernel<true, 16>);
        else if (pool_rows == 8) err = run(decode_compact_kernel<true, 8>);
        else err = run(decode_compact_kernel<true, 4>);
    } else {
        if (pool_rows == 32) err = run(decode_compact_kernel<false, 32>);
        else if (pool_rows == 24) err = run(decode_compact_kernel<false, 24>);
        else if (pool_rows == 16) err = run(decode_compact_kernel<false, 16>);
        else if (pool_rows == 8) err = run(decode_compact_kernel<false, 8>);
        else err = run(decode_compact_kernel<false, 4>);
    }
    if (err != cudaSuccess) return err;
    prof_mark_end(PROF_DECODE_COMPACT, stream);
    return cudaGetLastError();
}

cudaError_t launch_decode_dense(const DecodeArgs& a, const int* image_hw, double* out,
                                cudaStream_t stream)
{
    const HeadGeom& g = a.g;
    int dmax = 0;
    for (int l = 0; l < g.L; ++l) dmax = g.D[l] > dmax ? g.D[l] : dmax;
    const int row_floats = (dmax + 3) & ~3;
    const size_t smem = (size_t)(kDenseThreads / 8) * row_floats * 4;
    cudaError_t err = cudaFuncSetAttribute(decode_dense_kernel,
                                           cudaFuncAttributeMaxDynamicSharedMemorySize, (int)smem);
    if (err != cudaSuccess) return err;
    const long long rows = (long long)a.B * g.cells;
    long long grid = (rows + kDenseThreads / 8 - 1) / (kDenseThreads / 8);
    if (grid > 148 * 8) grid = 148 * 8;
    if (grid < 1) grid = 1;
    prof_mark_begin(PROF_OTHER, stream);
    decode_dense_kernel<<<(unsigned)grid, kDenseThreads, smem, stream>>>(a, image_hw, out, row_floats);
    prof_mark_end(PROF_OTHER, stream);
    return cudaGetLastError();
}
```

multigriddet_b200/engine.py:

```python
from __future__ import annotations

import ctypes

import numpy as np

from . import _lib

_NMS_METHODS = {"diou": _lib.NMS_DIOU, "standard": _lib.NMS_IOU, "iou": _lib.NMS_IOU,
                "cluster": _lib.NMS_IOU, "soft": _lib.NMS_SOFT, "wbf": _lib.NMS_WBF}


def _is_torch(x) -> bool:
    return type(x).__module__.split(".")[0] == "torch"


def _torch_stream(device_index: int) -> int:
    import torch
    return int(torch.cuda.current_stream(device_index).cuda_stream)


def _current_device() -> int:
    import sys
    torch = sys.modules.get("torch")
    if torch is not None and torch.cuda.is_available():
# ... 58 lines not shown
            raise ValueError(f"true_boxes must be (B, N, 5), got {boxes.shape}")
        B, N = boxes.shape[0], boxes.shape[1]
        if out is None:
            out = [_lib.pinned.empty((B, cfg.grid_h[l], cfg.grid_w[l],
                                      5 + cfg.num_anchors[l] + cfg.num_classes), np.float32)
                   for l in range(L)]
        ptrs = _lib.ptr_array([o.ctypes.data for o in out])
        rc = lib.mgd_encode_targets(ctypes.byref(cfg), ctypes.c_void_p(boxes.ctypes.data), B, N,
                                    ptrs, _lib.MEM_HOST, _current_device(), None,
                                    _lib.FLAG_SYNC | mode | (_lib.FLAG_HOST_ZEROCOPY if zerocopy else 0), stats)
    _lib.raise_for_status(rc)
    if return_stats:
        return out, {"n_valid_boxes": int(stats[0]), "n_skipped_writes": int(stats[1]),
                     "n_positive_cells": int(stats[2])}
    return out


def poll_status(device=None, stream=None):
    lib = _lib.load()
    dev = _current_device() if device is None else int(device)
    st = _torch_stream(dev) if stream is None else int(stream)
    _lib.raise_for_status(lib.mgd_poll_status(dev, ctypes.c_void_p(st)))



def _check_out(given, spec, B, device):
    import torch
    if "counts" not in given:
        raise ValueError("out= needs a 'counts' tensor")
    res = {}
    for k, t in given.items():
        shape, dt = ((B,), "int32") if k == "counts" else spec.get(k, (None, None))
        if shape is None:
            raise ValueError(f"out= has an unknown tensor {k!r}")
        dt = getattr(torch, dt) if isinstance(dt, str) else dt
        if not (_is_torch(t) and t.is_cuda and t.device == device and t.is_contiguous()
                and t.dtype == dt and tuple(t.shape) == tuple(shape)):
            raise ValueError(f"out[{k!r}] must be a contiguous {dt} CUDA tensor of shape {tuple(shape)}")
        res[k] = t
    return res


def decode_nms(preds, image_shapes, model_image_size, anchors, num_classes, max_boxes=100,
               confidence=0.1, nms_threshold=0.5, nms_method="diou", per_class=False,
               use_softmax=True, rescore_confidence=True, sync=True, return_stats=False,
               want=("boxes_xywh", "boxes_xyxy", "scores", "classes", "index"), out=None,
               zerocopy=False):
    lib = _lib.load()
    L = len(preds)
    if L != len(anchors):
        raise ValueError(f"Expected {len(anchors)} predictions, got {L}")
    grid_shapes = [(int(p.shape[1]), int(p.shape[2])) for p in preds]
    cfg = _lib.make_head_config(anchors, num_classes, model_image_size, grid_shapes)
    pc = post_config(max_boxes, confidence, nms_threshold, nms_method, per_class, use_softmax,
                     rescore_confidence)
    B = int(preds[0].shape[0])
    for l, p in enumerate(preds):
        exp = (B, cfg.grid_h[l], cfg.grid_w[l], 5 + cfg.num_anchors[l] + cfg.num_classes)
        if tuple(int(v) for v in p.shape) != exp:
            raise ValueError(f"preds[{l}] has shape {tuple(p.shape)}, expected {exp}")
    M = int(max_boxes)
    stats = (ctypes.c_longlong * 4)()
    hw = None
    d_hw = None
    if image_shapes is not None and _is_torch(image_shapes):
        import torch
        d_hw = image_shapes.to(torch.int32).contiguous()
        if tuple(d_hw.shape) != (B, 2) or not d_hw.is_cuda:
            raise ValueError("a tensor image_shapes must be a CUDA (B, 2) tensor")
    elif image_shapes is not None:
        hw = np.asarray(image_shapes, dtype=np.int32).reshape(-1, 2)
        if hw.shape[0] == 1 and B != 1:
            hw = np.tile(hw, (B, 1))
        if hw.shape[0] != B:
            raise ValueError(f"image_shapes must be (h, w) or (B, 2); got {hw.shape} for B={B}")
        hw = np.ascontiguousarray(hw)
    spec = {"boxes_xywh": ((B, M, 4), "float64"), "boxes_xyxy": ((B, M, 4), "int32"),
            "scores": ((B, M), "float64"), "classes": ((B, M), "int32"),
            "index": ((B, M), "int32")}
    given, out = out, {}
    if given is not None and not _is_torch(preds[0]):
        raise ValueError("out= is only supported with torch CUDA tensors")
    if _is_torch(preds[0]):
        import torch
        dev = preds[0].device.index or 0
        tp = [p.to(torch.float32).contiguous() for p in preds]
        if given is not None:
            out = _check_out(given, spec, B, tp[0].device)
        else:
            for k in want:
                out[k] = torch.empty(spec[k][0], dtype=getattr(torch, spec[k][1]), device=tp[0].device)
            out["counts"] = torch.empty((B,), dtype=torch.int32, device=tp[0].device)
        if d_hw is None and hw is not None:
            d_hw = torch.from_numpy(hw).to(tp[0].device, non_blocking=False)
        addr = lambda k: ctypes.c_void_p(out[k].data_ptr()) if k in out else None
        rc = lib.mgd_decode_nms(
            ctypes.byref(cfg), ctypes.byref(pc), _lib.ptr_array([p.data_ptr() for p in tp]), B,
            ctypes.c_void_p(d_hw.data_ptr()) if d_hw is not None else None,
            addr("boxes_xywh"), addr("boxes_xyxy"), addr("scores"), addr("classes"),
            addr("index"), addr("counts"), _lib.MEM_DEVICE, dev,
            ctypes.c_void_p(_torch_stream(dev)), _lib.FLAG_SYNC if sync else 0, stats)
        out["_keepalive"] = (tp, d_hw)
    else:
        npreds = [np.ascontiguousarray(np.asarray(p), dtype=np.float32) for p in preds]
        for k in want:
            out[k] = _lib.pinned.empty(spec[k][0], spec[k][1])
        out["counts"] = np.empty((B,), dtype=np.int32)
        addr = lambda k: ctypes.c_void_p(out[k].ctypes.data) if k in out else None
        rc = lib.mgd_decode_nms(
            ctypes.byref(cfg), ctypes.byref(pc), _lib.ptr_array([p.ctypes.data for p in npreds]), B,
            ctypes.c_void_p(hw.ctypes.data) if hw is not None else None,
            addr("boxes_xywh"), addr("boxes_xyxy"), addr("scores"), addr("classes"),
            addr("index"), addr("counts"), _lib.MEM_HOST, _current_device(), None,
            _lib.FLAG_SYNC | (_lib.FLAG_HOST_ZEROCOPY if zerocopy else 0), stats)
    _lib.raise_for_status(rc)
    if not sync:
        return out
    out.pop("_keepalive", None)
    if return_stats:
        out["stats"] = {"n_candidates": int(stats[0]), "n_detections": int(stats[1])}
    return out


def grid_step(true_boxes, y_true, preds, image_shapes, input_shape, anchors, num_classes,
              max_boxes=100, confidence=0.1, nms_threshold=0.5, nms_method="diou", per_class=False,
              use_softmax=True, rescore_confidence=True, sync=True,
              want=("boxes_xywh", "boxes_xyxy", "scores", "classes", "index"), out=None):
    import torch
    lib = _lib.load()
    if len(preds) != len(anchors) or len(y_true) != len(anchors):
        raise ValueError(f"Expected {len(anchors)} tensors per list")
    grid_shapes = [(int(p.shape[1]), int(p.shape[2])) for p in preds]
    cfg = _lib.make_head_config(anchors, num_classes, input_shape, grid_shapes)
    pc = post_config(max_boxes, confidence, nms_threshold, nms_method, per_class, use_softmax,
                     rescore_confidence)
    B = int(preds[0].shape[0])
    Be, N = int(true_boxes.shape[0]), int(true_boxes.shape[1])
    dev = preds[0].device.index or 0
    for l, (p, y) in enumerate(zip(preds, y_true)):
        d = 5 + cfg.num_anchors[l] + cfg.num_classes
        if tuple(p.shape) != (B, cfg.grid_h[l], cfg.grid_w[l], d) or \
                tuple(y.shape) != (Be, cfg.grid_h[l], cfg.grid_w[l], d):
            raise ValueError(f"layer {l}: unexpected tensor shape")
        if not (p.is_cuda and y.is_cuda and p.is_contiguous() and y.is_contiguous()
                and p.dtype == torch.float32 and y.dtype == torch.float32):
            raise ValueError("grid_step takes contiguous float32 CUDA tensors")
    tb = true_boxes.to(torch.float32).contiguous()
    d_hw = None
    if image_shapes is not None:
        d_hw = image_shapes if _is_torch(image_shapes) else torch.from_numpy(
            np.ascontiguousarray(np.broadcast_to(np.asarray(image_shapes, np.int32).reshape(-1, 2), (B, 2)))).to(preds[0].device)
        d_hw = d_hw.to(torch.int32).contiguous()
    M = int(max_boxes)
    spec = {"boxes_xywh": ((B, M, 4), torch.float64), "boxes_xyxy": ((B, M, 4), torch.int32),
            "scores": ((B, M), torch.float64), "classes": ((B, M), torch.int32),
            "index": ((B, M), torch.int32)}
    if out is not None:
        out = _check_out(out, spec, B, preds[0].device)
    else:
        out = {k: torch.empty(spec[k][0], dtype=spec[k][1], device=preds[0].device) for k in want}
        out["counts"] = torch.empty((B,), dtype=torch.int32, device=preds[0].device)
    addr = lambda k: ctypes.c_void_p(out[k].data_ptr()) if k in out else None
    rc = lib.mgd_encode_decode_nms(
        ctypes.byref(cfg), ctypes.byref(pc), ctypes.c_void_p(tb.data_ptr()), Be, N,
        _lib.ptr_array([y.data_ptr() for y in y_true]),
        _lib.ptr_array([p.data_ptr() for p in preds]), B,
        ctypes.c_void_p(d_hw.data_ptr()) if d_hw is not None else None,
        addr("boxes_xywh"), addr("boxes_xyxy"), addr("scores"), addr("classes"), addr("index"),
        addr("counts"), dev, ctypes.c_void_p(_torch_stream(dev)), _lib.FLAG_SYNC if sync else 0)
    _lib.raise_for_status(rc)
    if not sync:
        out["_keepalive"] = (tb, d_hw)
    return out


def decode_dense(preds, anchors, num_classes, model_image_size, image_shapes=None,
                 use_softmax=True, rescore_confidence=True):
    lib = _lib.load()
    if len(preds) != len(anchors):
        raise ValueError(f"Expected {len(anchors)} predictions, got {len(preds)}")
    grid_shapes = [(int(p.shape[1]), int(p.shape[2])) for p in preds]
    cfg = _lib.make_head_config(anchors, num_classes, model_image_size, grid_shapes)
    pc = post_config(use_softmax=use_softmax, rescore_confidence=rescore_confidence)
    B = int(preds[0].shape[0])
    cells = sum(g[0] * g[1] for g in grid_shapes)
    hw = None
    if image_shapes is not None:
        hw = np.asarray(image_shapes, dtype=np.int32).reshape(-1, 2)
        if hw.shape[0] == 1 and B != 1:
            hw = np.tile(hw, (B, 1))
        hw = np.ascontiguousarray(hw)
    if _is_torch(preds[0]):
        import torch
        dev = preds[0].device.index or 0
        tp = [p.to(torch.float32).contiguous() for p in preds]
        out = torch.empty((B, cells, 5 + int(num_classes)), dtype=torch.float64, device=tp[0].device)
        d_hw = torch.from_numpy(hw).to(tp[0].device) if hw is not None else None
        rc = lib.mgd_decode_dense(ctypes.byref(cfg), ctypes.byref(pc),
                                  _lib.ptr_array([p.data_ptr() for p in tp]), B,
                                  ctypes.c_void_p(d_hw.data_ptr()) if d_hw is not None else None,
                                  ctypes.c_void_p(out.data_ptr()), _lib.MEM_DEVICE, dev,
                                  ctypes.c_void_p(_torch_stream(dev)), _lib.FLAG_SYNC)
    else:
        npreds = [np.ascontiguousarray(np.asarray(p), dtype=np.float32) for p in preds]
        out = np.empty((B, cells, 5 + int(num_classes)), dtype=np.float64)
        rc = lib.mgd_decode_dense(ctypes.byref(cfg), ctypes.byref(pc),
                                  _lib.ptr_array([p.ctypes.data for p in npreds]), B,
                                  ctypes.c_void_p(hw.ctypes.data) if hw is not None else None,
                                  ctypes.c_void_p(out.ctypes.data), _lib.MEM_HOST,
                                  _current_device(), None, _lib.FLAG_SYNC)
    _lib.raise_for_status(rc)
    return out


_WBF_CONF = {"avg": 0, "max": 1, "box_and_model_avg": 2, "absent_model_aware_avg": 2}


def wbf(boxes, scores, classes, box_weights=None, iou_thr=0.55, skip_box_thr=0.0, conf_type="avg"):
    lib = _lib.load()
    b = np.ascontiguousarray(np.asarray(boxes, dtype=np.float64).reshape(-1, 4))
    s = np.ascontiguousarray(np.asarray(scores, dtype=np.float64).reshape(-1))
    c = np.ascontiguousarray(np.asarray(classes).astype(np.int32).reshape(-1))
    n = b.shape[0]
    if s.shape[0] != n or c.shape[0] != n:
        raise ValueError("boxes, scores and classes disagree on n")
    w = None
    if box_weights is not None:
        w = np.ascontiguousarray(np.asarray(box_weights, dtype=np.float64).reshape(-1))
    ob = np.empty((max(n, 1), 4), dtype=np.float64)
    osc = np.empty((max(n, 1),), dtype=np.float64)
    oc = np.empty((max(n, 1),), dtype=np.int32)
    n_out = ctypes.c_int(0)
    rc = lib.mgd_wbf(ctypes.c_void_p(b.ctypes.data), ctypes.c_void_p(s.ctypes.data),
                     ctypes.c_void_p(c.ctypes.data),
                     ctypes.c_void_p(w.ctypes.data) if w is not None else None, n, float(iou_thr),
                     float(skip_box_thr), _WBF_CONF.get(conf_type, 0), ctypes.c_void_p(ob.ctypes.data),
                     ctypes.c_void_p(osc.ctypes.data), ctypes.c_void_p(oc.ctypes.data),
                     ctypes.cast(ctypes.byref(n_out), ctypes.c_void_p), _lib.MEM_HOST,
                     _current_device(), None, _lib.FLAG_SYNC)
    _lib.raise_for_status(rc)
    k = n_out.value
    return ob[:k].copy(), osc[:k].copy(), oc[:k].copy()


def soft_nms(boxes, scores, sigma=0.5, score_threshold=0.001):
    lib = _lib.load()
    b = np.ascontiguousarray(np.asarray(boxes, dtype=np.float64).reshape(-1, 4))
    s = np.ascontiguousarray(np.asarray(scores, dtype=np.float64).reshape(-1))
    n = b.shape[0]
    if s.shape[0] != n:
        raise ValueError("boxes and scores disagree on n")
    keep = np.empty((max(n, 1),), dtype=np.int32)
    soft = np.empty((max(n, 1),), dtype=np.float64)
    n_keep = ctypes.c_int(0)
    rc = lib.mgd_soft_nms(ctypes.c_void_p(b.ctypes.data), ctypes.c_void_p(s.ctypes.data), n,
                          float(sigma), float(score_threshold), ctypes.c_void_p(keep.ctypes.data),
                          ctypes.c_void_p(soft.ctypes.data),
                          ctypes.cast(ctypes.byref(n_keep), ctypes.c_void_p), _lib.MEM_HOST,
                          _current_device(), None, _lib.FLAG_SYNC)
    _lib.raise_for_status(rc)
    k = n_keep.value
    return keep[:k].astype(np.int64), soft[:k].copy()


def nms(boxes, scores, classes=None, nms_threshold=0.5, nms_method="diou", per_class=False,
        max_keep=0):
    lib = _lib.load()
    if nms_method not in _NMS_METHODS or nms_method in ("soft", "wbf"):
        raise NotImplementedError(f"nms_method={nms_method!r} is not a greedy hard NMS")
    b = np.ascontiguousarray(np.asarray(boxes, dtype=np.float64).reshape(-1, 4))
    s = np.ascontiguousarray(np.asarray(scores, dtype=np.float64).reshape(-1))
    n = b.shape[0]
    if s.shape[0] != n:
        raise ValueError("boxes and scores disagree on n")
    c = None
    if classes is not None:
        c = np.ascontiguousarray(np.asarray(classes).astype(np.int32).reshape(-1))
    keep = np.empty((max(n, 1),), dtype=np.int32)
    n_keep = ctypes.c_int(0)
    rc = lib.mgd_nms(ctypes.c_void_p(b.ctypes.data), ctypes.c_void_p(s.ctypes.data),
                     ctypes.c_void_p(c.ctypes.data) if c is not None else None, n,
                     float(nms_threshold), _NMS_METHODS[nms_method], int(bool(per_class)),
                     int(max_keep), ctypes.c_void_p(keep.ctypes.data),
                     ctypes.cast(ctypes.byref(n_keep), ctypes.c_void_p), _lib.MEM_HOST,
                     _current_device(), None, _lib.FLAG_SYNC)
    _lib.raise_for_status(rc)
    return keep[:n_keep.value].astype(np.int64)


PROFILE_KINDS = ("encode_assign", "encode_fill", "decode_compact", "nms", "other")


def profile_begin():
    _lib.raise_for_status(_lib.load().mgd_profile_begin())


def profile_end():
    ms = (ctypes.c_double * len(PROFILE_KINDS))()
    n = (ctypes.c_longlong * len(PROFILE_KINDS))()
    _lib.raise_for_status(_lib.load().mgd_profile_end(ms, n))
    return {k: (float(ms[i]), int(n[i])) for i, k in enumerate(PROFILE_KINDS)}



def match_detections(det_boxes, det_scores, det_classes, det_counts, gt_boxes, gt_classes, gt_counts,
                     iou_thresholds, iou_mode="corner", return_matched=False, sync=True):
    lib = _lib.load()
    mode = {"corner": _lib.IOU_CORNER, "centre": _lib.IOU_CENTRE, "center": _lib.IOU_CENTRE}[iou_mode]
    thr = np.ascontiguousarray(np.asarray(iou_thresholds, dtype=np.float64).reshape(-1))
    T = int(thr.shape[0])
    thr_p = thr.ctypes.data_as(ctypes.POINTER(ctypes.c_double))
    if _is_torch(det_boxes):
        import torch
        dev = det_boxes.device
        f64 = lambda x: x.to(device=dev, dtype=torch.float64).contiguous()
        i32 = lambda x: x.to(device=dev, dtype=torch.int32).contiguous()
        db, ds, dc, dn = f64(det_boxes), f64(det_scores), i32(det_classes), i32(det_counts)
        gb, gc, gn = f64(gt_boxes), i32(gt_classes), i32(gt_counts)
        B, M, N = int(ds.shape[0]), int(ds.shape[1]), int(gc.shape[1])
        tp = torch.empty((T, B, M), dtype=torch.uint8, device=dev)
        who = torch.empty((T, B, M), dtype=torch.int32, device=dev) if return_matched else None
        p = lambda x: ctypes.c_void_p(x.data_ptr()) if x is not None and x.numel() else None
        idx = dev.index or 0
        rc = lib.mgd_match_detections(p(db), p(ds), p(dc), p(dn), B, M, p(gb), p(gc), p(gn), N, thr_p, T,
                                      mode, p(tp), p(who), _lib.MEM_DEVICE, idx,
                                      ctypes.c_void_p(_torch_stream(idx)), _lib.FLAG_SYNC if sync else 0)
    else:
        f64 = lambda x: np.ascontiguousarray(np.asarray(x), dtype=np.float64)
        i32 = lambda x: np.ascontiguousarray(np.asarray(x), dtype=np.int32)
        db, ds, dc, dn = f64(det_boxes), f64(det_scores), i32(det_classes), i32(det_counts)
        gb, gc, gn = f64(gt_boxes), i32(gt_classes), i32(gt_counts)
        B, M, N = ds.shape[0], ds.shape[1], gc.shape[1]
        tp = np.zeros((T, B, M), dtype=np.uint8)
        who = np.full((T, B, M), -1, dtype=np.int32) if return_matched else None
        p = lambda x: ctypes.c_void_p(x.ctypes.data) if x is not None and x.size else None
        rc = lib.mgd_match_detections(p(db), p(ds), p(dc), p(dn), B, M, p(gb), p(gc), p(gn), N, thr_p, T,
                                      mode, p(tp), p(who), _lib.MEM_HOST, _current_device(), None,
                                      _lib.FLAG_SYNC)
    _lib.raise_for_status(rc)
    return (tp, who) if return_matched else tp


def iou_matrix(boxes1, boxes2):
    lib = _lib.load()
    b1 = np.ascontiguousarray(np.asarray(boxes1, dtype=np.float64).reshape(-1, 4))
    b2 = np.ascontiguousarray(np.asarray(boxes2, dtype=np.float64).reshape(-1, 4))
    out = np.zeros((b1.shape[0], b2.shape[0]), dtype=np.float64)
    if out.size:
        rc = lib.mgd_iou_matrix(ctypes.c_void_p(b1.ctypes.data), b1.shape[0],
                                ctypes.c_void_p(b2.ctypes.data), b2.shape[0],
                                ctypes.c_void_p(out.ctypes.data), _lib.MEM_HOST, _current_device(),
                                None, _lib.FLAG_SYNC)
        _lib.raise_for_status(rc)
    return out



def reshape_boxes_batch(boxes, params, counts=None, want_f32=True, sync=True):
    lib = _lib.load()
    if _is_torch(boxes):
        import torch
        dev = boxes.device
        i32 = boxes.dtype == torch.int32
        b = boxes.contiguous() if i32 else boxes.to(torch.float64).contiguous()
        B, N = int(b.shape[0]), int(b.shape[1])
        par = torch.as_tensor(params).to(device=dev, dtype=torch.int32).contiguous()
        cnt = None if counts is None else torch.as_tensor(counts).to(device=dev, dtype=torch.int32).contiguous()
        out = torch.empty_like(b)
        o32 = torch.empty((B, N, 5), dtype=torch.float32, device=dev) if want_f32 else None
        ocn = torch.empty((B,), dtype=torch.int32, device=dev)
        p = lambda x: ctypes.c_void_p(x.data_ptr()) if x is not None and x.numel() else None
        idx = dev.index or 0
        rc = lib.mgd_reshape_boxes(p(b), _lib.BOXES_I32 if i32 else _lib.BOXES_F64, p(cnt), p(par), B, N,
                                   p(out), p(o32), p(ocn), _lib.MEM_DEVICE, idx,
                                   ctypes.c_void_p(_torch_stream(idx)), _lib.FLAG_SYNC if sync else 0)
    else:
        b = np.asarray(boxes)
        i32 = b.dtype == np.int32
        b = np.ascontiguousarray(b, dtype=np.int32 if i32 else np.float64)
        B, N = b.shape[0], b.shape[1]
        par = np.ascontiguousarray(np.asarray(params), dtype=np.int32).reshape(B, 10)
        cnt = None if counts is None else np.ascontiguousarray(np.asarray(counts), dtype=np.int32)
        out = np.zeros_like(b)
        o32 = np.zeros((B, N, 5), dtype=np.float32) if want_f32 else None
        ocn = np.zeros((B,), dtype=np.int32)
        p = lambda x: ctypes.c_void_p(x.ctypes.data) if x is not None and x.size else None
        rc = lib.mgd_reshape_boxes(p(b), _lib.BOXES_I32 if i32 else _lib.BOXES_F64, p(cnt), p(par), B, N,
                                   p(out), p(o32), p(ocn), _lib.MEM_HOST, _current_device(), None,
                                   _lib.FLAG_SYNC)
    _lib.raise_for_status(rc)
    return out, o32, ocn


def letterbox_boxes_batch(boxes, src_shapes, input_shape, max_boxes_per_image, counts=None,
                          expansion=1, multiscale_shapes=None, hflip=None, sync=True):
    lib = _lib.load()
    B, N = int(boxes.shape[0]), int(boxes.shape[1])
    par = np.zeros((B, 6), dtype=np.int32)
    par[:, 0:2] = np.asarray(src_shapes, dtype=np.int64).reshape(B, 2)
    if multiscale_shapes is not None:
        par[:, 2:4] = np.asarray(multiscale_shapes, dtype=np.int64).reshape(B, 2)
    if hflip is not None:
        par[:, 4] = np.asarray(hflip).astype(np.int32).reshape(B)
    cap = int(max_boxes_per_image) * int(expansion)
    ih, iw = int(input_shape[0]), int(input_shape[1])
    if _is_torch(boxes):
        import torch
        dev = boxes.device
        b = boxes.to(torch.float32).contiguous()
        d_par = torch.from_numpy(par).to(dev)
        cnt = None if counts is None else torch.as_tensor(counts).to(device=dev, dtype=torch.int32).contiguous()
        out = torch.empty((B, cap, 5), dtype=torch.float32, device=dev)
        p = lambda x: ctypes.c_void_p(x.data_ptr()) if x is not None and x.numel() else None
        idx = dev.index or 0
        rc = lib.mgd_letterbox_boxes(p(b), p(cnt), p(d_par), B, N, ih, iw, int(max_boxes_per_image),
                                     int(expansion), p(out), _lib.MEM_DEVICE, idx,
                                     ctypes.c_void_p(_torch_stream(idx)), _lib.FLAG_SYNC if sync else 0)
    else:
        b = np.ascontiguousarray(np.asarray(boxes), dtype=np.float32)
        cnt = None if counts is None else np.ascontiguousarray(np.asarray(counts), dtype=np.int32)
        out = np.zeros((B, cap, 5), dtype=np.float32)
        p = lambda x: ctypes.c_void_p(x.ctypes.data) if x is not None and x.size else None
        rc = lib.mgd_letterbox_boxes(p(b), p(cnt), p(par), B, N, ih, iw, int(max_boxes_per_image),
                                     int(expansion), p(out), _lib.MEM_HOST, _current_device(), None,
                                     _lib.FLAG_SYNC)
    _lib.raise_for_status(rc)
    return out


def mosaic_merge_boxes_batch(boxes, sample_index, crop_xy, image_size, want_f32=True, sync=True):
    lib = _lib.load()
    H, W = int(image_size[0]), int(image_size[1])
    if _is_torch(boxes):
        import torch
        dev = boxes.device
        b = boxes.to(torch.float64).contiguous()
        n_src, N = int(b.shape[0]), int(b.shape[1])
        par = torch.cat([torch.as_tensor(sample_index).reshape(-1, 4).to(dev),
                         torch.as_tensor(crop_xy).reshape(-1, 2).to(dev)], 1).to(torch.int32).contiguous()
        B = int(par.shape[0])
        out = torch.empty((B, N, 5), dtype=torch.float64, device=dev)
        o32 = torch.empty((B, N, 5), dtype=torch.float32, device=dev) if want_f32 else None
        ocn = torch.empty((B,), dtype=torch.int32, device=dev)
        p = lambda x: ctypes.c_void_p(x.data_ptr()) if x is not None and x.numel() else None
        idx = dev.index or 0
        rc = lib.mgd_mosaic_merge_boxes(p(b), n_src, N, p(par), B, H, W, p(out), p(o32), p(ocn),
                                        _lib.MEM_DEVICE, idx, ctypes.c_void_p(_torch_stream(idx)),
                                        _lib.FLAG_SYNC if sync else 0)
    else:
        b = np.ascontiguousarray(np.asarray(boxes), dtype=np.float64)
        n_src, N = b.shape[0], b.shape[1]
        par = np.ascontiguousarray(np.concatenate([np.asarray(sample_index).reshape(-1, 4),
                                                   np.asarray(crop_xy).reshape(-1, 2)], 1), dtype=np.int32)
        B = par.shape[0]
        out = np.zeros((B, N, 5), dtype=np.float64)
        o32 = np.zeros((B, N, 5), dtype=np.float32) if want_f32 else None
        ocn = np.zeros((B,), dtype=np.int32)
        p = lambda x: ctypes.c_void_p(x.ctypes.data) if x is not None and x.size else None
        rc = lib.mgd_mosaic_merge_boxes(p(b), n_src, N, p(par), B, H, W, p(out), p(o32), p(ocn),
                                        _lib.MEM_HOST, _current_device(), None, _lib.FLAG_SYNC)
    _lib.raise_for_status(rc)
    return out, o32, ocn



def ignore_masks(y_preds, y_trues, anchors, input_shape, num_classes, ignore_thresh=0.5, eps=1e-7,
                 sync=True):
    lib = _lib.load()
    L = len(y_preds)
    grids = [(int(p.shape[1]), int(p.shape[2])) for p in y_preds]
    cfg = _lib.make_head_config([np.asarray(a, dtype=np.float32) for a in anchors], num_classes,
                                input_shape, grids)
    B = int(y_preds[0].shape[0])
    outs = []
    if _is_torch(y_preds[0]):
        import torch
        dev = y_preds[0].device
        yp = [t.to(torch.float32).contiguous() for t in y_preds]
        yt = [t.to(device=dev, dtype=torch.float32).contiguous() for t in y_trues]
        for gh, gw in grids:
            outs.append(tuple(torch.empty((B, gh, gw, 1), dtype=torch.float32, device=dev) for _ in range(3)))
        ptr = lambda ts: _lib.ptr_array([t.data_ptr() for t in ts])
        idx = dev.index or 0
        rc = lib.mgd_ignore_mask(ctypes.byref(cfg), ptr(yp), ptr(yt), B, float(ignore_thresh), float(eps),
                                 ptr([o[0] for o in outs]), ptr([o[1] for o in outs]), ptr([o[2] for o in outs]),
                                 _lib.MEM_DEVICE, idx, ctypes.c_void_p(_torch_stream(idx)),
                                 _lib.FLAG_SYNC if sync else 0)
    else:
        yp = [np.ascontiguousarray(np.asarray(t), dtype=np.float32) for t in y_preds]
        yt = [np.ascontiguousarray(np.asarray(t), dtype=np.float32) for t in y_trues]
        for gh, gw in grids:
            outs.append(tuple(np.zeros((B, gh, gw, 1), dtype=np.float32) for _ in range(3)))
        ptr = lambda ts: _lib.ptr_array([t.ctypes.data for t in ts])
        rc = lib.mgd_ignore_mask(ctypes.byref(cfg), ptr(yp), ptr(yt), B, float(ignore_thresh), float(eps),
                                 ptr([o[0] for o in outs]), ptr([o[1] for o in outs]), ptr([o[2] for o in outs]),
                                 _lib.MEM_HOST, _current_device(), None, _lib.FLAG_SYNC)
    _lib.raise_for_status(rc)
    return outs


def encode_ignore_masks(true_boxes, y_preds, anchors, input_shape, num_classes, ignore_thresh=0.5,
                        eps=1e-7, want_y_true=True, sync=True, semantics="numpy"):
    import torch
    lib = _lib.load()
    grids = [(int(p.shape[1]), int(p.shape[2])) for p in y_preds]
    cfg = _lib.make_head_config([np.asarray(a, dtype=np.float32) for a in anchors], num_classes,
                                input_shape, grids)
    dev = y_preds[0].device
    B, N = int(true_boxes.shape[0]), int(true_boxes.shape[1])
    tb = true_boxes.to(device=dev, dtype=torch.float32).contiguous()
    yp = [t.to(torch.float32).contiguous() for t in y_preds]
    yt = [torch.empty_like(t) for t in yp] if want_y_true else None
    outs = [tuple(torch.empty((B, gh, gw, 1), dtype=torch.float32, device=dev) for _ in range(3))
            for gh, gw in grids]
    ptr = lambda ts: _lib.ptr_array([t.data_ptr() for t in ts])
    idx = dev.index or 0
    flags = (_lib.FLAG_SYNC if sync else 0) | (_lib.FLAG_TF_COMPAT if semantics == "tf_compat" else 0)
    rc = lib.mgd_encode_ignore_mask(ctypes.byref(cfg), ctypes.c_void_p(tb.data_ptr()), B, N, ptr(yp),
                                    ptr(yt) if yt is not None else None, float(ignore_thresh), float(eps),
                                    ptr([o[0] for o in outs]), ptr([o[1] for o in outs]),
                                    ptr([o[2] for o in outs]), idx, ctypes.c_void_p(_torch_stream(idx)), flags)
    _lib.raise_for_status(rc)
    return yt, outs
```

Baseline: 1.392 million.

## Let blocked decode producer warps steal and consume published slots

Pulls the consumer slot-processing body out into a reusable consume_slot function. When a producer warp is blocked waiting for a free slot, it can now claim the next published slot through a CAS on next_seq and process it itself instead of sleeping. After the producers finish, they also join the consumer loop. Stealing is on by default (MGD_DECODE_STEAL), which adds shared-memory atomics and register pressure on producer warps. The change also adds optional clock-based wait statistics under a debug flag and a new shape option.

```diff
diff --git a/include/mgd.h b/include/mgd.h
--- a/include/mgd.h
+++ b/include/mgd.h
@@ -156,6 +156,9 @@
 MGD_API int mgd_profile_begin(void);
 MGD_API int mgd_profile_end(double *ms, long long *launches);
 
+#define MGD_DECODE_WAIT_STATS 4
+MGD_API int mgd_decode_wait_stats(int device, unsigned long long *out);
+
 struct DLTensor;
 MGD_API int mgd_encode_targets_dlpack(const mgd_head_config *cfg, const struct DLTensor *boxes,
                               struct DLTensor *const *y_true, void *stream, int flags,
diff --git a/multigriddet_b200/_lib.py b/multigriddet_b200/_lib.py
--- a/multigriddet_b200/_lib.py
+++ b/multigriddet_b200/_lib.py
@@ -67,7 +67,8 @@
            "mgd_host_free", "mgd_release_workspace", "mgd_reshape_boxes", "mgd_mosaic_merge_boxes",
            "mgd_ignore_mask", "mgd_encode_decode_nms", "mgd_letterbox_boxes",
            "mgd_encode_ignore_mask", "mgd_exchange_create", "mgd_exchange_connect",
-           "mgd_exchange_buffer", "mgd_exchange_timeouts", "mgd_exchange_destroy")
+           "mgd_exchange_buffer", "mgd_exchange_timeouts", "mgd_exchange_destroy",
+           "mgd_decode_wait_stats")
 
 IPC_HANDLE_BYTES = 64
 
@@ -191,6 +192,8 @@
     lib.mgd_profile_begin.restype = ctypes.c_int
     lib.mgd_profile_end.restype = ctypes.c_int
     lib.mgd_profile_end.argtypes = [_DP, _LLP]
+    lib.mgd_decode_wait_stats.restype = ctypes.c_int
+    lib.mgd_decode_wait_stats.argtypes = [ctypes.c_int, ctypes.POINTER(ctypes.c_ulonglong)]
     _lib = lib
     return lib
 
diff --git a/multigriddet_b200/csrc/api.cu b/multigriddet_b200/csrc/api.cu
--- a/multigriddet_b200/csrc/api.cu
+++ b/multigriddet_b200/csrc/api.cu
@@ -981,6 +981,17 @@
     }
     t_prof_spans.clear();
     return rc;
+}
+
+int mgd_decode_wait_stats(int device, unsigned long long* out)
+{
+    if (!out) return fail(MGD_ERR_INVALID_ARGUMENT, "mgd_decode_wait_stats: out is null");
+    int num_sms;
+    DeviceScope dev_scope;
+    int rc = prepare_device(device, &num_sms, &dev_scope);
+    if (rc) return rc;
+    CUDA_TRY(decode_wait_stats(out));
+    return MGD_OK;
 }
 
 int mgd_poll_status(int device, void* stream)
diff --git a/multigriddet_b200/csrc/common.cuh b/multigriddet_b200/csrc/common.cuh
--- a/multigriddet_b200/csrc/common.cuh
+++ b/multigriddet_b200/csrc/common.cuh
@@ -65,6 +65,7 @@
     int* counts;
     int chunk_blocks;
     int debug;
+    int steal;
 };
 
 #define MGD_MAX_MIRRORS 7
@@ -179,6 +180,7 @@
 cudaError_t launch_encode_fill(const EncodeArgs& a, int num_sms, cudaStream_t stream,
                                bool overlap_previous = false);
 cudaError_t launch_decode(const DecodeArgs& a, int num_sms, cudaStream_t stream);
+cudaError_t decode_wait_stats(unsigned long long* out);
 cudaError_t launch_nms(const NmsArgs& a, int num_sms, cudaStream_t stream);
 size_t encode_assign_smem_bytes(const HeadGeom& g, int N);
 bool encode_needs_big_tables(const HeadGeom& g, int N);
diff --git a/multigriddet_b200/csrc/decode.cu b/multigriddet_b200/csrc/decode.cu
--- a/multigriddet_b200/csrc/decode.cu
+++ b/multigriddet_b200/csrc/decode.cu
@@ -356,11 +356,263 @@
     int* fill_seq;
     int* next_seq;
     int* producers_done;
+    unsigned long long* wait;
     int stride;
 };
 
-template <class Sh>
-__device__ __forceinline__ void producer(const DecodeArgs& a, const GroupShared& gs, int p, int P)
+constexpr int kWaitStats = 4;
+__device__ unsigned long long g_wait_stats[kWaitStats];
+
+__device__ __forceinline__ int ld_volatile_smem(const int* p)
+{
+    int v;
+    asm volatile("ld.volatile.shared.s32 %0, [%1];" : "=r"(v) : "r"(smem_u32(p)) : "memory");
+    return v;
+}
+
+template <class Sh, int kC>
+__device__ __forceinline__ bool consume_slot(const DecodeArgs& a, const GroupShared& gs,
+                                             const uint32_t* tab, int seq)
+{
+    constexpr int kSlots = Sh::kSlots;
+    constexpr int kRows = Sh::kRows;
+    constexpr int kSplit = 32 / kRows;
+    const HeadGeom& g = a.g;
+    const int lane = threadIdx.x & 31;
+    const int j = lane & 7;
+    const int oct = lane >> 3;
+    const bool softmax = a.use_softmax != 0;
+    const bool rescore = a.rescore != 0;
+    const int C = kC ? kC : g.C;
+    const int body = C >= 8 ? (C & ~7) : 0;
+    const int tail = C - body;
+    constexpr float kNear = 0.99999f;
+    constexpr float kNearD = -1.1e-5f;
+
+    const int slot = seq % kSlots;
+    mbar_wait(&gs.full[slot], ((unsigned)(seq / kSlots)) & 1u);
+    const SlotMeta& meta = gs.meta[slot];
+    const int count = meta.count;
+    if (count < 0) {
+        __syncwarp();
+        if (lane == 0) st_release_smem(&gs.released[slot], seq / kSlots + 1);
+        return false;
+    }
+    const int layer = meta.layer;
+    const float* rows = gs.rows + (size_t)slot * kRows * gs.stride;
+
+    const int lrow = lane & (kRows - 1), part = lane / kRows;
+    bool pass = lrow < count && !(a.debug & 4);
+    float mc = -INFINITY, sum = 0.f;
+    if (pass) {
+        const float4* c4 = reinterpret_cast<const float4*>(rows + (size_t)lrow * gs.stride + 8);
+        const int n4 = C / 4, per = (n4 + kSplit - 1) / kSplit;
+        const int i0 = part * per, i1 = min(n4, i0 + per);
+        if (softmax && rescore) {
+            #pragma unroll 4
+            for (int i = i0; i < i1; ++i) {
+                const float4 v = c4[i];
+                mc = fmaxf(fmaxf(mc, fmaxf(v.x, v.y)), fmaxf(v.z, v.w));
+                sum += (fast_exp(v.x) + fast_exp(v.y)) + (fast_exp(v.z) + fast_exp(v.w));
+            }
+        } else {
+            #pragma unroll 4
+            for (int i = i0; i < i1; ++i) {
+                const float4 v = c4[i];
+                mc = fmaxf(fmaxf(mc, fmaxf(v.x, v.y)), fmaxf(v.z, v.w));
+            }
+        }
+    }
+    if (kSplit == 2) {
+        mc = fmaxf(mc, __shfl_xor_sync(0xffffffffu, mc, 16));
+        sum += __shfl_xor_sync(0xffffffffu, sum, 16);
+    }
+    if (pass && rescore) {
+        if (softmax) {
+            float ub = __fdividef(meta.bound[lrow] * fast_exp(mc), sum);
+            if (!(sum < 3.0e38f) || !(ub == ub)) ub = 3.0e38f;
+            pass = ub >= a.score_lo;
+        } else {
+            pass = meta.bound[lrow] * fast_sigmoid(mc) >= a.score_lo;
+        }
+    }
+    unsigned todo = __ballot_sync(0xffffffffu, pass) & (kRows == 32 ? 0xffffffffu : (1u << (kRows & 31)) - 1u);
+    if (a.debug & 2) todo = 0;
+
+    unsigned cand_rows = 0;
+    while (todo) {
+        const unsigned pos = nth_set_bit(todo, oct);
+        const bool live = pos < 32u;
+        const unsigned posr = live ? pos : (unsigned)__ffs((int)todo) - 1u;
+        const float* x = rows + (size_t)posr * gs.stride;
+        const float mx = __shfl_sync(0xffffffffu, mc, (int)posr);
+        const float4 head = *reinterpret_cast<const float4*>(x + 4);
+        const int l0 = oct * 8;
+        float pa, pc, obj;
+        int ka, kc;
+        if (softmax) {
+            const float ma = fmaxf(head.y, fmaxf(head.z, head.w));
+            const float logit = x[5 + (j < 2 ? j : 2)];
+            const float da = __fsub_rn(logit, ma);
+            const float arg = j < 3 ? (da < -104.0f ? -104.0f : da) : (j == 3 ? -head.x : 0.f);
+            const float ea = expf_full2(arg, tab);
+
+            const float* cx = x + 8;
+            float r = 0.f, e_tail = 0.f;
+            int near_cnt = 0, near_first = INT_MAX;
+            if (body) {
+                #pragma unroll 10
+                for (int i = j; i < body; i += 8) {
+                    const float d = __fsub_rn(cx[i], mx);
+                    const float e = expf_core2(d < -104.0f ? -104.0f : d, tab);
+                    r = __fadd_rn(r, e);
+                    near_track(d, kNearD, i, near_first, near_cnt);
+                }
+                r = __fadd_rn(r, __shfl_xor_sync(0xffffffffu, r, 1));
+                r = __fadd_rn(r, __shfl_xor_sync(0xffffffffu, r, 2));
+                r = __fadd_rn(r, __shfl_xor_sync(0xffffffffu, r, 4));
+            }
+            if (tail) {
+                if (j < tail) {
+                    const float d = __fsub_rn(cx[body + j], mx);
+                    e_tail = expf_core2(d < -104.0f ? -104.0f : d, tab);
+                    near_track(d, kNearD, body + j, near_first, near_cnt);
+                }
+                for (int k = 0; k < tail; ++k)
+                    r = __fadd_rn(r, __shfl_sync(0xffffffffu, e_tail, l0 + k));
+            }
+            pc = __frcp_rn(r);
+            const float e0 = __shfl_sync(0xffffffffu, ea, l0);
+            const float e1 = __shfl_sync(0xffffffffu, ea, l0 + 1);
+            const float e2 = __shfl_sync(0xffffffffu, ea, l0 + 2);
+            const float eo = __shfl_sync(0xffffffffu, ea, l0 + 3);
+            const float sa = __fadd_rn(__fadd_rn(__fadd_rn(0.f, e0), e1), e2);
+            pa = __frcp_rn(sa);
+            obj = __frcp_rn(__fadd_rn(1.0f, eo));
+            const unsigned has = (__ballot_sync(0xffffffffu, near_cnt > 0) >> l0) & 0xffu;
+            const unsigned many = (__ballot_sync(0xffffffffu, near_cnt > 1) >> l0) & 0xffu;
+            const bool simple = !many && __popc(has) == 1;
+            kc = __shfl_sync(0xffffffffu, near_first, l0 + (has ? __ffs((int)has) - 1 : 0));
+            const int n0 = e0 >= kNear, n1 = e1 >= kNear, n2 = e2 >= kNear;
+            ka = n0 ? 0 : (n1 ? 1 : 2);
+            if (__any_sync(0xffffffffu, !simple || n0 + n1 + n2 != 1)) {
+                int first = INT_MAX;
+                for (int i = j; i < C; i += 8) {
+                    const float d = __fsub_rn(cx[i], mx);
+                    const float e = expf_core2(d < -104.0f ? -104.0f : d, tab);
+                    if (e >= kNear && __fdiv_rn(e, r) == pc) { first = i; break; }
+                }
+                first = min(first, __shfl_xor_sync(0xffffffffu, first, 1));
+                first = min(first, __shfl_xor_sync(0xffffffffu, first, 2));
+                first = min(first, __shfl_xor_sync(0xffffffffu, first, 4));
+                if (!simple) kc = first;
+                if (n0 + n1 + n2 != 1) {
+                    ka = INT_MAX;
+                    if (n2 && __fdiv_rn(e2, sa) == pa) ka = 2;
+                    if (n1 && __fdiv_rn(e1, sa) == pa) ka = 1;
+                    if (n0 && __fdiv_rn(e0, sa) == pa) ka = 0;
+                }
+            }
+        } else {
+            float best = -INFINITY;
+            int first = INT_MAX;
+            for (int i = j; i < C; i += 8) {
+                const float qv = __fdiv_rn(1.0f, __fadd_rn(1.0f, expf_full2(-x[8 + i], tab)));
+                if (qv > best) { best = qv; first = i; }
+            }
+            #pragma unroll
+            for (int d = 1; d <= 4; d <<= 1) {
+                const float ob = __shfl_xor_sync(0xffffffffu, best, d);
+                const int oi = __shfl_xor_sync(0xffffffffu, first, d);
+                if (ob > best || (ob == best && oi < first)) { best = ob; first = oi; }
+            }
+            pc = best; kc = first;
+            const float logit = j == 0 ? head.x : (j == 1 ? head.y : (j == 2 ? head.z : head.w));
+            const float qv = __fdiv_rn(1.0f, __fadd_rn(1.0f, expf_full2(-logit, tab)));
+            obj = __shfl_sync(0xffffffffu, qv, l0);
+            const float q0 = __shfl_sync(0xffffffffu, qv, l0 + 1);
+            const float q1 = __shfl_sync(0xffffffffu, qv, l0 + 2);
+            const float q2 = __shfl_sync(0xffffffffu, qv, l0 + 3);
+            pa = -INFINITY; ka = INT_MAX;
+            if (q0 > pa) { pa = q0; ka = 0; }
+            if (q1 > pa) { pa = q1; ka = 1; }
+            if (q2 > pa) { pa = q2; ka = 2; }
+        }
+        float score = obj;
+        if (rescore) score = __fmul_rn(__fmul_rn(score, pa), pc);
+        const bool is_cand = live && j == 0 && (double)score >= a.confidence;
+        __syncwarp();
+        if (is_cand) {
+            float4 res;
+            res.x = score;
+            res.y = __int_as_float(kc);
+            res.z = __int_as_float(g.anchor_first[layer] + ka);
+            res.w = 0.f;
+            *reinterpret_cast<float4*>(const_cast<float*>(x) + 4) = res;
+        }
+        cand_rows |= __reduce_or_sync(0xffffffffu, is_cand ? (1u << pos) : 0u);
+        #pragma unroll
+        for (int q = 0; q < 4; ++q) todo &= todo - 1;
+    }
+    __syncwarp();
+    const bool mine = lane < kRows && ((cand_rows >> lane) & 1u);
+    float4 t = make_float4(0.f, 0.f, 0.f, 0.f), res = t;
+    unsigned grow = 0;
+    if (mine) {
+        const float* x = rows + (size_t)lane * gs.stride;
+        t = *reinterpret_cast<const float4*>(x);
+        res = *reinterpret_cast<const float4*>(x + 4);
+        grow = (unsigned)meta.row[lane];
+    }
+    if (cand_rows) asm volatile("fence.proxy.async.shared::cta;" ::: "memory");
+    __syncwarp();
+    if (lane == 0) {
+        st_release_smem(&gs.released[slot], seq / kSlots + 1);
+        if (a.debug & 8) atomicAdd(&gs.wait[3], 1ull);
+    }
+    if (cand_rows) {
+        const unsigned long long magic = a.cells_magic[layer];
+        const unsigned b = magic ? (unsigned)__umul64hi((unsigned long long)grow, magic) : grow;
+        const unsigned same = __match_any_sync(0xffffffffu, mine ? b : (0x80000000u | (unsigned)lane));
+        const int leader = __ffs((int)same) - 1;
+        int base = 0;
+        if (mine && lane == leader) base = atomicAdd(a.counts + b, __popc(same));
+        base = __shfl_sync(0xffffffffu, base, leader);
+        if (mine) {
+            Cand cd;
+            cd.score = res.x;
+            cd.index = g.cell_off[layer] + (int)(grow - b * (unsigned)(g.gh[layer] * g.gw[layer]));
+            cd.t[0] = t.x; cd.t[1] = t.y; cd.t[2] = t.z; cd.t[3] = t.w;
+            cd.cls = __float_as_int(res.y);
+            cd.anchor = __float_as_int(res.z);
+            a.cand[(size_t)b * g.cells + base + __popc(same & ((1u << lane) - 1u))] = cd;
+        }
+    }
+    return true;
+}
+
+template <class Sh, int kC>
+__device__ __forceinline__ void consumer(const DecodeArgs& a, const GroupShared& gs,
+                                         const uint32_t* tab)
+{
+    constexpr int kSlots = Sh::kSlots;
+    const int lane = threadIdx.x & 31;
+    for (;;) {
+        int seq = 0;
+        if (lane == 0) {
+            seq = atomicAdd(gs.next_seq, 1);
+            const unsigned t0 = (a.debug & 8) ? (unsigned)clock() : 0u;
+            while (ld_acquire_smem(&gs.published[seq % kSlots]) != seq) __nanosleep(40);
+            if (a.debug & 8) atomicAdd(&gs.wait[1], (unsigned long long)((unsigned)clock() - t0));
+        }
+        seq = __shfl_sync(0xffffffffu, seq, 0);
+        if (!consume_slot<Sh, kC>(a, gs, tab, seq)) break;
+    }
+}
+
+template <class Sh, int kC>
+__device__ __forceinline__ void producer(const DecodeArgs& a, const GroupShared& gs, const uint32_t* tab,
+                                         int p, int P)
 {
     constexpr int kSlots = Sh::kSlots;
     constexpr int kRows = Sh::kRows;
@@ -374,14 +626,34 @@
     int seq = 0, slot = 0, count = 0;
     bool have_slot = false;
 
-    auto acquire = [&]() {
-        if (lane == 0) {
-            seq = atomicAdd(gs.fill_seq, 1);
-            const int use = seq / kSlots;
-            while (ld_acquire_smem(&gs.released[seq % kSlots]) != use) __nanosleep(40);
-        }
+    auto acquire = [&](bool steal) {
+        if (lane == 0) seq = atomicAdd(gs.fill_seq, 1);
         seq = __shfl_sync(0xffffffffu, seq, 0);
         slot = seq % kSlots;
+        const int use = seq / kSlots;
+        unsigned t0 = (a.debug & 8) ? (unsigned)clock() : 0u;
+        for (;;) {
+            int n = -1;
+            if (lane == 0) {
+                if (ld_acquire_smem(&gs.released[slot]) == use) {
+                    n = -2;
+                } else if (steal) {
+                    n = ld_volatile_smem(gs.next_seq);
+                    if (ld_acquire_smem(&gs.published[n % kSlots]) != n || atomicCAS(gs.next_seq, n, n + 1) != n)
+                        n = -1;
+                }
+                if (n == -1) __nanosleep(40);
+            }
+            n = __shfl_sync(0xffffffffu, n, 0);
+            if (n == -1) continue;
+            if ((a.debug & 8) && lane == 0) {
+                atomicAdd(&gs.wait[0], (unsigned long long)((unsigned)clock() - t0));
+                if (n >= 0) atomicAdd(&gs.wait[2], 1ull);
+            }
+            if (n == -2) break;
+            consume_slot<Sh, kC>(a, gs, tab, n);
+            if (a.debug & 8) t0 = (unsigned)clock();
+        }
         have_slot = true;
     };
     auto publish = [&](int cnt, int layer) {
@@ -413,7 +685,7 @@
         auto stage_rows = [&](int blk, unsigned todo, float bound) {
             const int row = blk * 32 + lane;
             while (todo) {
-                if (!have_slot) acquire();
+                if (!have_slot) acquire(a.steal != 0);
                 const int free_slots = kRows - count;
                 const int rank = __popc(todo & ((1u << lane) - 1u));
                 const bool take = ((todo >> lane) & 1u) && rank < free_slots;
@@ -468,231 +740,10 @@
     if (lane == 0) done = atomicAdd(gs.producers_done, 1) + 1;
     done = __shfl_sync(0xffffffffu, done, 0);
     if (done == kProducers)
-        for (int c = 0; c < kConsumers; ++c) {
-            acquire();
+        for (int c = 0; c < (a.steal ? kConsumers + kProducers : kConsumers); ++c) {
+            acquire(false);
             publish(-1, 0);
         }
-}
-
-template <class Sh, int kC>
-__device__ __forceinline__ void consumer(const DecodeArgs& a, const GroupShared& gs,
-                                         const uint32_t* tab)
-{
-    constexpr int kSlots = Sh::kSlots;
-    constexpr int kRows = Sh::kRows;
-    constexpr int kSplit = 32 / kRows;
-    const HeadGeom& g = a.g;
-    const int lane = threadIdx.x & 31;
-    const int j = lane & 7;
-    const int oct = lane >> 3;
-    const bool softmax = a.use_softmax != 0;
-    const bool rescore = a.rescore != 0;
-    const int C = kC ? kC : g.C;
-    const int body = C >= 8 ? (C & ~7) : 0;
-    const int tail = C - body;
-    constexpr float kNear = 0.99999f;
-    constexpr float kNearD = -1.1e-5f;
-
-    for (;;) {
-        int seq = 0;
-        if (lane == 0) {
-            seq = atomicAdd(gs.next_seq, 1);
-            while (ld_acquire_smem(&gs.published[seq % kSlots]) != seq) __nanosleep(40);
-        }
-        seq = __shfl_sync(0xffffffffu, seq, 0);
-        const int slot = seq % kSlots;
-        mbar_wait(&gs.full[slot], ((unsigned)(seq / kSlots)) & 1u);
-        const SlotMeta& meta = gs.meta[slot];
-        const int count = meta.count;
-        if (count < 0) break;
-        const int layer = meta.layer;
-        const float* rows = gs.rows + (size_t)slot * kRows * gs.stride;
-
-        const int lrow = lane & (kRows - 1), part = lane / kRows;
-        bool pass = lrow < count && !(a.debug & 4);
-        float mc = -INFINITY, sum = 0.f;
-        if (pass) {
-            const float4* c4 = reinterpret_cast<const float4*>(rows + (size_t)lrow * gs.stride + 8);
-            const int n4 = C / 4, per = (n4 + kSplit - 1) / kSplit;
-            const int i0 = part * per, i1 = min(n4, i0 + per);
-            if (softmax && rescore) {
-                #pragma unroll 4
-                for (int i = i0; i < i1; ++i) {
-                    const float4 v = c4[i];
-                    mc = fmaxf(fmaxf(mc, fmaxf(v.x, v.y)), fmaxf(v.z, v.w));
-                    sum += (fast_exp(v.x) + fast_exp(v.y)) + (fast_exp(v.z) + fast_exp(v.w));
-                }
-            } else {
-                #pragma unroll 4
-                for (int i = i0; i < i1; ++i) {
-                    const float4 v = c4[i];
-                    mc = fmaxf(fmaxf(mc, fmaxf(v.x, v.y)), fmaxf(v.z, v.w));
-                }
-            }
-        }
-        if (kSplit == 2) {
-            mc = fmaxf(mc, __shfl_xor_sync(0xffffffffu, mc, 16));
-            sum += __shfl_xor_sync(0xffffffffu, sum, 16);
-        }
-        if (pass && rescore) {
-            if (softmax) {
-                float ub = __fdividef(meta.bound[lrow] * fast_exp(mc), sum);
-                if (!(sum < 3.0e38f) || !(ub == ub)) ub = 3.0e38f;
-                pass = ub >= a.score_lo;
-            } else {
-                pass = meta.bound[lrow] * fast_sigmoid(mc) >= a.score_lo;
-            }
-        }
-        unsigned todo = __ballot_sync(0xffffffffu, pass) & (kRows == 32 ? 0xffffffffu : (1u << (kRows & 31)) - 1u);
-        if (a.debug & 2) todo = 0;
-
-        unsigned cand_rows = 0;
-        while (todo) {
-            const unsigned pos = nth_set_bit(todo, oct);
-            const bool live = pos < 32u;
-            const unsigned posr = live ? pos : (unsigned)__ffs((int)todo) - 1u;
-            const float* x = rows + (size_t)posr * gs.stride;
-            const float mx = __shfl_sync(0xffffffffu, mc, (int)posr);
-            const float4 head = *reinterpret_cast<const float4*>(x + 4);
-            const int l0 = oct * 8;
-            float pa, pc, obj;
-            int ka, kc;
-            if (softmax) {
-                const float ma = fmaxf(head.y, fmaxf(head.z, head.w));
-                const float logit = x[5 + (j < 2 ? j : 2)];
-                const float da = __fsub_rn(logit, ma);
-                const float arg = j < 3 ? (da < -104.0f ? -104.0f : da) : (j == 3 ? -head.x : 0.f);
-                const float ea = expf_full2(arg, tab);
-
-                const float* cx = x + 8;
-                float r = 0.f, e_tail = 0.f;
-                int near_cnt = 0, near_first = INT_MAX;
-                if (body) {
-                    #pragma unroll 10
-                    for (int i = j; i < body; i += 8) {
-                        const float d = __fsub_rn(cx[i], mx);
-                        const float e = expf_core2(d < -104.0f ? -104.0f : d, tab);
-                        r = __fadd_rn(r, e);
-                        near_track(d, kNearD, i, near_first, near_cnt);
-                    }
-                    r = __fadd_rn(r, __shfl_xor_sync(0xffffffffu, r, 1));
-                    r = __fadd_rn(r, __shfl_xor_sync(0xffffffffu, r, 2));
-                    r = __fadd_rn(r, __shfl_xor_sync(0xffffffffu, r, 4));
-                }
-                if (tail) {
-                    if (j < tail) {
-                        const float d = __fsub_rn(cx[body + j], mx);
-                        e_tail = expf_core2(d < -104.0f ? -104.0f : d, tab);
-                        near_track(d, kNearD, body + j, near_first, near_cnt);
-                    }
-                    for (int k = 0; k < tail; ++k)
-                        r = __fadd_rn(r, __shfl_sync(0xffffffffu, e_tail, l0 + k));
-                }
-                pc = __frcp_rn(r);
-                const float e0 = __shfl_sync(0xffffffffu, ea, l0);
-                const float e1 = __shfl_sync(0xffffffffu, ea, l0 + 1);
-                const float e2 = __shfl_sync(0xffffffffu, ea, l0 + 2);
-                const float eo = __shfl_sync(0xffffffffu, ea, l0 + 3);
-                const float sa = __fadd_rn(__fadd_rn(__fadd_rn(0.f, e0), e1), e2);
-                pa = __frcp_rn(sa);
-                obj = __frcp_rn(__fadd_rn(1.0f, eo));
-                const unsigned has = (__ballot_sync(0xffffffffu, near_cnt > 0) >> l0) & 0xffu;
-                const unsigned many = (__ballot_sync(0xffffffffu, near_cnt > 1) >> l0) & 0xffu;
-                const bool simple = !many && __popc(has) == 1;
-                kc = __shfl_sync(0xffffffffu, near_first, l0 + (has ? __ffs((int)has) - 1 : 0));
-                const int n0 = e0 >= kNear, n1 = e1 >= kNear, n2 = e2 >= kNear;
-                ka = n0 ? 0 : (n1 ? 1 : 2);
-                if (__any_sync(0xffffffffu, !simple || n0 + n1 + n2 != 1)) {
-                    int first = INT_MAX;
-                    for (int i = j; i < C; i += 8) {
-                        const float d = __fsub_rn(cx[i], mx);
-                        const float e = expf_core2(d < -104.0f ? -104.0f : d, tab);
-                        if (e >= kNear && __fdiv_rn(e, r) == pc) { first = i; break; }
-                    }
-                    first = min(first, __shfl_xor_sync(0xffffffffu, first, 1));
-                    first = min(first, __shfl_xor_sync(0xffffffffu, first, 2));
-                    first = min(first, __shfl_xor_sync(0xffffffffu, first, 4));
-                    if (!simple) kc = first;
-                    if (n0 + n1 + n2 != 1) {
-                        ka = INT_MAX;
-                        if (n2 && __fdiv_rn(e2, sa) == pa) ka = 2;
-                        if (n1 && __fdiv_rn(e1, sa) == pa) ka = 1;
-                        if (n0 && __fdiv_rn(e0, sa) == pa) ka = 0;
-                    }
-                }
-            } else {
-                float best = -INFINITY;
-                int first = INT_MAX;
-                for (int i = j; i < C; i += 8) {
-                    const float qv = __fdiv_rn(1.0f, __fadd_rn(1.0f, expf_full2(-x[8 + i], tab)));
-                    if (qv > best) { best = qv; first = i; }
-                }
-                #pragma unroll
-                for (int d = 1; d <= 4; d <<= 1) {
-                    const float ob = __shfl_xor_sync(0xffffffffu, best, d);
-                    const int oi = __shfl_xor_sync(0xffffffffu, first, d);
-                    if (ob > best || (ob == best && oi < first)) { best = ob; first = oi; }
-                }
-                pc = best; kc = first;
-                const float logit = j == 0 ? head.x : (j == 1 ? head.y : (j == 2 ? head.z : head.w));
-                const float qv = __fdiv_rn(1.0f, __fadd_rn(1.0f, expf_full2(-logit, tab)));
-                obj = __shfl_sync(0xffffffffu, qv, l0);
-                const float q0 = __shfl_sync(0xffffffffu, qv, l0 + 1);
-                const float q1 = __shfl_sync(0xffffffffu, qv, l0 + 2);
-                const float q2 = __shfl_sync(0xffffffffu, qv, l0 + 3);
-                pa = -INFINITY; ka = INT_MAX;
-                if (q0 > pa) { pa = q0; ka = 0; }
-                if (q1 > pa) { pa = q1; ka = 1; }
-                if (q2 > pa) { pa = q2; ka = 2; }
-            }
-            float score = obj;
-            if (rescore) score = __fmul_rn(__fmul_rn(score, pa), pc);
-            const bool is_cand = live && j == 0 && (double)score >= a.confidence;
-            __syncwarp();
-            if (is_cand) {
-                float4 res;
-                res.x = score;
-                res.y = __int_as_float(kc);
-                res.z = __int_as_float(g.anchor_first[layer] + ka);
-                res.w = 0.f;
-                *reinterpret_cast<float4*>(const_cast<float*>(x) + 4) = res;
-            }
-            cand_rows |= __reduce_or_sync(0xffffffffu, is_cand ? (1u << pos) : 0u);
-            #pragma unroll
-            for (int q = 0; q < 4; ++q) todo &= todo - 1;
-        }
-        __syncwarp();
-        const bool mine = lane < kRows && ((cand_rows >> lane) & 1u);
-        float4 t = make_float4(0.f, 0.f, 0.f, 0.f), res = t;
-        unsigned grow = 0;
-        if (mine) {
-            const float* x = rows + (size_t)lane * gs.stride;
-            t = *reinterpret_cast<const float4*>(x);
-            res = *reinterpret_cast<const float4*>(x + 4);
-            grow = (unsigned)meta.row[lane];
-        }
-        if (cand_rows) asm volatile("fence.proxy.async.shared::cta;" ::: "memory");
-        __syncwarp();
-        if (lane == 0) st_release_smem(&gs.released[slot], seq / kSlots + 1);
-        if (cand_rows) {
-            const unsigned long long magic = a.cells_magic[layer];
-            const unsigned b = magic ? (unsigned)__umul64hi((unsigned long long)grow, magic) : grow;
-            const unsigned same = __match_any_sync(0xffffffffu, mine ? b : (0x80000000u | (unsigned)lane));
-            const int leader = __ffs((int)same) - 1;
-            int base = 0;
-            if (mine && lane == leader) base = atomicAdd(a.counts + b, __popc(same));
-            base = __shfl_sync(0xffffffffu, base, leader);
-            if (mine) {
-                Cand cd;
-                cd.score = res.x;
-                cd.index = g.cell_off[layer] + (int)(grow - b * (unsigned)(g.gh[layer] * g.gw[layer]));
-                cd.t[0] = t.x; cd.t[1] = t.y; cd.t[2] = t.z; cd.t[3] = t.w;
-                cd.cls = __float_as_int(res.y);
-                cd.anchor = __float_as_int(res.z);
-                a.cand[(size_t)b * g.cells + base + __popc(same & ((1u << lane) - 1u))] = cd;
-            }
-        }
-    }
 }
 
 template <class Sh, int kC>
@@ -706,7 +757,7 @@
     __shared__ SlotMeta s_meta[kSlots];
     __shared__ uint32_t s_tab[2 * MGD_EXP2F_N];
     __shared__ int s_counters[3];
-
+    __shared__ unsigned long long s_wait[kWaitStats];
 
     const int tid = threadIdx.x;
     const int warp = tid >> 5;
@@ -721,6 +772,7 @@
             s_released[sl] = 0;
         }
         s_counters[0] = s_counters[1] = s_counters[2] = 0;
+        for (int k = 0; k < kWaitStats; ++k) s_wait[k] = 0;
         fence_mbar_init();
     }
     __syncthreads();
@@ -738,11 +790,16 @@
     gs.fill_seq = &s_counters[0];
     gs.next_seq = &s_counters[1];
     gs.producers_done = &s_counters[2];
+    gs.wait = s_wait;
     gs.stride = stride;
     if (pw >= 0)
-        producer<Sh>(a, gs, blockIdx.x * kProducers + pw, gridDim.x * kProducers);
-    else
+        producer<Sh, kC>(a, gs, s_tab, blockIdx.x * kProducers + pw, gridDim.x * kProducers);
+    if (pw < 0 || a.steal)
         consumer<Sh, kC>(a, gs, s_tab);
+    if (a.debug & 8) {
+        __syncthreads();
+        if (tid < kWaitStats) atomicAdd(&g_wait_stats[tid], s_wait[tid]);
+    }
 }
 
 }
@@ -837,6 +894,8 @@
     static int env_debug = -1;
     if (env_debug < 0) { const char* e = getenv("MGD_DECODE_DEBUG"); env_debug = e ? atoi(e) : 0; }
     a.debug = env_debug;
+    const char* env_steal = getenv("MGD_DECODE_STEAL");
+    a.steal = env_steal ? atoi(env_steal) != 0 : 1;
     if (fast && g.C <= 128 && !env_impl) {
         long long blocks = 0;
         for (int l = 0; l < g.L; ++l) blocks += (a.rows_in_layer[l] + 31) / 32;
@@ -872,6 +931,7 @@
         else if (env_shape == 3) err = run(ws::Shape<3, 8, 17, 16, 8>());
         else if (env_shape == 4) err = run(ws::Shape<3, 6, 7, 32>());
         else if (env_shape == 5) err = run(ws::Shape<2, 4, 8, 32>());
+        else if (env_shape == 6) err = run(ws::Shape<4, 6, 16, 16, 8>());
         else err = run(ws::Shape<3, 7, 17, 16, 8>());
         if (err != cudaErrorInvalidConfiguration) return err;
         cudaGetLastError();
@@ -919,6 +979,14 @@
     return cudaGetLastError();
 }
 
+cudaError_t decode_wait_stats(unsigned long long* out)
+{
+    cudaError_t e = cudaMemcpyFromSymbol(out, ws::g_wait_stats, sizeof(ws::g_wait_stats));
+    if (e != cudaSuccess) return e;
+    const unsigned long long zero[ws::kWaitStats] = {};
+    return cudaMemcpyToSymbol(ws::g_wait_stats, zero, sizeof(zero));
+}
+
 cudaError_t launch_decode_dense(const DecodeArgs& a, const int* image_hw, double* out,
                                 cudaStream_t stream)
 {
diff --git a/multigriddet_b200/engine.py b/multigriddet_b200/engine.py
--- a/multigriddet_b200/engine.py
+++ b/multigriddet_b200/engine.py
@@ -384,6 +384,16 @@
     return {k: (float(ms[i]), int(n[i])) for i, k in enumerate(PROFILE_KINDS)}
 
 
+DECODE_WAIT_STATS = ("producer_blocked_cycles", "consumer_wait_cycles", "stolen_slots", "slots")
+
+
+def decode_wait_stats(device=None):
+    out = (ctypes.c_ulonglong * len(DECODE_WAIT_STATS))()
+    dev = _current_device() if device is None else device
+    _lib.raise_for_status(_lib.load().mgd_decode_wait_stats(dev, out))
+    return {k: int(out[i]) for i, k in enumerate(DECODE_WAIT_STATS)}
+
+
 
 def match_detections(det_boxes, det_scores, det_classes, det_counts, gt_boxes, gt_classes, gt_counts,
                      iou_thresholds, iou_mode="corner", return_matched=False, sync=True):
```

New measurement: 1.221 million, median of 6. -12.3%, worse.
